# pecos/tps

Measured on AMD Instinct MI355X. Metric: DG RHS evals/sec (MDOF/s) for 3D p=3 reacting cyl at 1/2/4/8 MI355X, higher is better.
Workload: dtype f64

## Files before the change

### include/tpsrhs.h

```cpp
#ifndef TPSRHS_H_
#define TPSRHS_H_

#include <stdint.h>

#ifdef __cplusplus
extern "C" {
#endif

#define TPSRHS_MAXDIM 3
#define TPSRHS_MAXSPECIES 8
#define TPSRHS_MAXEQUATIONS (TPSRHS_MAXDIM + 2 + TPSRHS_MAXSPECIES)
#define TPSRHS_MAXREACTIONS 34
#define TPSRHS_MAXCHEMPARAMS 3
#define TPSRHS_MAXTABLE 1000
#define TPSRHS_MAXORDER 5

enum tpsrhs_status {
  TPSRHS_OK = 0,
  TPSRHS_ERR_INVALID_ARGUMENT = 1,
  TPSRHS_ERR_UNSUPPORTED = 2,
  TPSRHS_ERR_MESH = 3,
  TPSRHS_ERR_DEVICE = 4,
  TPSRHS_ERR_NO_DEVICE = 5,
  TPSRHS_ERR_HALO = 6
// ... 148 lines not shown
} tpsrhs_chemistry;

typedef struct tpsrhs_radiation {
  int model;
  tpsrhs_table nec_table;
} tpsrhs_radiation;

enum tpsrhs_sgs_model { TPSRHS_SGS_NONE = 0, TPSRHS_SGS_SMAGORINSKY = 1, TPSRHS_SGS_SIGMA = 2 };
typedef struct tpsrhs_sgs {
  int model_type;
  double model_const;
  double model_floor;
} tpsrhs_sgs;
typedef struct tpsrhs_visc_sponge {
  int enabled;
  double normal[3], point[3];
  double width, ratio;
} tpsrhs_visc_sponge;

typedef struct tpsrhs_lte {
  tpsrhs_table energy_table;
  tpsrhs_table gas_constant_table;
  tpsrhs_table sound_speed_table;
  tpsrhs_table viscosity_table;
  tpsrhs_table conductivity_table;
  tpsrhs_table electric_conductivity_table;
} tpsrhs_lte;

typedef struct tpsrhs_physics {
  int eq_system;
  int working_fluid;
  tpsrhs_dry_air dry_air;
  tpsrhs_perfect_mixture mixture;
  int transport_model;
  tpsrhs_constant_transport constant_transport;
  tpsrhs_gas_transport gas_transport;
  tpsrhs_chemistry chemistry;
  tpsrhs_radiation radiation;
  tpsrhs_sgs sgs;
  tpsrhs_visc_sponge visc_sponge;
  tpsrhs_lte lte;
} tpsrhs_physics;

typedef struct tpsrhs_bc {
  int attribute;
  int category;
  int type;
  double data[4 + TPSRHS_MAXSPECIES];
} tpsrhs_bc;

typedef int (*tpsrhs_halo_fn)(void *ctx, int phase, const double *send, double *recv,
                              int num_neighbors, const int *neighbor_ranks,
                              const int64_t *send_offsets, const int64_t *recv_offsets, void *stream);

enum tpsrhs_reduce_op { TPSRHS_REDUCE_SUM = 0, TPSRHS_REDUCE_MIN = 1 };
typedef int (*tpsrhs_reduce_fn)(void *ctx, double *values, int count, int op, void *stream);

typedef struct tpsrhs_runtime {
  int device;
  void *stream;
  tpsrhs_halo_fn halo;
  void *halo_ctx;
  tpsrhs_reduce_fn reduce;
  void *reduce_ctx;
} tpsrhs_runtime;

typedef struct tpsrhs_operator *tpsrhs_handle;

int tpsrhs_create(const tpsrhs_mesh *mesh, const tpsrhs_disc *disc, const tpsrhs_physics *physics,
                  int num_bcs, const tpsrhs_bc *bcs, const tpsrhs_runtime *runtime,
                  tpsrhs_handle *out);

int tpsrhs_destroy(tpsrhs_handle h);

int tpsrhs_mult(tpsrhs_handle h, const double *x, double *y, double time, double *max_char_speed);

int tpsrhs_mult_host(tpsrhs_handle h, const double *x, double *y, double time,
                     double *max_char_speed);

int tpsrhs_update_gradients(tpsrhs_handle h, const double *x);

int tpsrhs_get_primitives(tpsrhs_handle h, double *up_out);
int tpsrhs_get_gradients(tpsrhs_handle h, double *gradup_out);
int tpsrhs_get_plasma_conductivity(tpsrhs_handle h, const double *x, double *sigma_out);

enum tpsrhs_point_quantity {
  TPSRHS_POINT_PRIMITIVES = 0,
  TPSRHS_POINT_PRESSURE = 1,
  TPSRHS_POINT_SOUND_SPEED = 2,
  TPSRHS_POINT_MAX_CHAR_SPEED = 3
};
int tpsrhs_eval_pointwise(tpsrhs_handle h, int quantity, int64_t n, const double *U, double *out);

int tpsrhs_table_eval(const tpsrhs_table *table, int64_t n, const double *x, double *f);

int tpsrhs_math_eval(int function, int64_t n, const double *x, double *y);

int64_t tpsrhs_height(tpsrhs_handle h);
int64_t tpsrhs_num_dofs(tpsrhs_handle h);
int tpsrhs_num_equation(tpsrhs_handle h);

int tpsrhs_enable_kernel_timing(tpsrhs_handle h, int enable);
int tpsrhs_kernel_times(tpsrhs_handle h, int capacity, const char **names, double *milliseconds);
int tpsrhs_mult_times(tpsrhs_handle h, int capacity, double *milliseconds);

int tpsrhs_kernel_bytes(tpsrhs_handle h, int capacity, const char **names, double *bytes);

int tpsrhs_rk4_step(tpsrhs_handle h, double *x, double *time, double dt, double *max_char_speed, int64_t *nan_count);

int tpsrhs_advance(tpsrhs_handle h, double *x, double *time, double *dt, int num_steps, int constant_dt, double cfl,
                   double hmin, int64_t *nan_count);

int tpsrhs_set_dt(tpsrhs_handle h, double dt);

#define TPSRHS_MAXHEATSOURCES 4
#define TPSRHS_MAXSPONGEZONES 2
#define TPSRHS_MAXPASSIVESCALARS 4

typedef struct tpsrhs_heat_source {
  double value;
  double radius, point1[3], point2[3];
} tpsrhs_heat_source;

enum tpsrhs_sponge_type { TPSRHS_SPONGE_PLANAR = 0, TPSRHS_SPONGE_ANNULUS = 1 };
enum tpsrhs_sponge_solution { TPSRHS_SPONGE_USERDEF = 0, TPSRHS_SPONGE_MIXEDOUT = 1 };

typedef struct tpsrhs_sponge_zone {
  int type;
  int solution_type;
  double tol;
  double normal[3], point0[3], point_init[3];
  double r1, r2;
  double mult_factor;
  double target_U[TPSRHS_MAXEQUATIONS];
} tpsrhs_sponge_zone;

typedef struct tpsrhs_passive_scalar {
  double coords[3];
  double radius;
  double value;
} tpsrhs_passive_scalar;

typedef struct tpsrhs_forcing {
  int has_pressure_gradient;
  double pressure_gradient[3];
  int num_heat_sources;
  tpsrhs_heat_source heat_sources[TPSRHS_MAXHEATSOURCES];
  int num_sponge_zones;
  tpsrhs_sponge_zone sponge_zones[TPSRHS_MAXSPONGEZONES];
  int num_passive_scalars;
  tpsrhs_passive_scalar passive_scalars[TPSRHS_MAXPASSIVESCALARS];
} tpsrhs_forcing;

int tpsrhs_set_forcing(tpsrhs_handle h, const tpsrhs_forcing *forcing);

typedef struct tpsrhs_mixing_length {
  double max_mixing_length;
  double pr_ratio;
  double lewis;
  double bulk_multiplier;
} tpsrhs_mixing_length;
int tpsrhs_set_mixing_length(tpsrhs_handle h, const double *distance, const tpsrhs_mixing_length *params);

int tpsrhs_set_joule_heating(tpsrhs_handle h, const double *joule_heating);

int tpsrhs_face_tables(const tpsrhs_mesh *mesh, int num_bcs, const tpsrhs_bc *bcs, int32_t *face_nbr,
// ... 11 lines not shown
```

### tps_amd/capi.py

```python
from __future__ import annotations

import ctypes as C
import os

import numpy as np

MAXDIM = 3
MAXSPECIES = 8
MAXEQUATIONS = MAXDIM + 2 + MAXSPECIES
MAXREACTIONS = 34
MAXCHEMPARAMS = 3
NUM_GASPARAMS = 4

EULER, NS, NS_PASSIVE = 0, 1, 2
DRY_AIR, USER_DEFINED, LTE_FLUID = 0, 1, 2
ARGON_MINIMAL, ARGON_MIXTURE, CONSTANT = 0, 1, 2
ARRHENIUS, HOFFERTLIEN, TABULATED_RXN = 0, 1, 2
NONE_RAD, NET_EMISSION = 0, 1
SPECIES_MW, SPECIES_CHARGES, FORMATION_ENERGY, SPECIES_DEGENERACY = 0, 1, 2, 3
CLMB_ATT, CLMB_REP, AR_AR1P, AR_E, AR_AR, NONE_ARGCOLL = 0, 1, 2, 3, 4, 5
INLET, OUTLET, WALL = 0, 1, 2
SUB_DENS_VEL, SUB_DENS_VEL_NR, SUB_VEL_CONST_ENT = 2, 6, 7
SUB_DENS_VEL_FACE_X, SUB_DENS_VEL_FACE_Y, SUB_DENS_VEL_FACE_Z = 3, 4, 5
SUB_P, SUB_P_NR, SUB_MF_NR, SUB_MF_NR_PW = 0, 2, 3, 4
# ... 452 lines not shown
    for sp in range(nsp):
        mx.gas_params[sp + SPECIES_MW * nsp] = mw[sp]
        mx.gas_params[sp + SPECIES_CHARGES * nsp] = -1.0 if sp == 3 else 0.0
        mx.gas_params[sp + FORMATION_ENERGY * nsp] = 0.0
        mx.gas_params[sp + SPECIES_DEGENERACY * nsp] = 1.0
        mx.molar_cv[sp] = cv[sp]
    ph.transport_model = CONSTANT
    ph.constant_transport.electron_index = 3
    ph.chemistry.electron_index = 3
    ph.chemistry.num_reactions = 0
    ph._keep = []
    return ph


def make_bc(attribute, category, bc_type, data=()) -> BC:
    bc = BC()
    bc.attribute, bc.category, bc.type = attribute, category, bc_type
    for i, v in enumerate(data):
        bc.data[i] = float(v)
    return bc


class MeshArgs:

    def __init__(self, hm):
        self.ev = np.ascontiguousarray(hm.elem_vertices, dtype=np.int32)
        self.ex = np.ascontiguousarray(hm.elem_coords, dtype=np.float64)
        self.bv = np.ascontiguousarray(hm.bdr_vertices, dtype=np.int32)
        self.ba = np.ascontiguousarray(hm.bdr_attributes, dtype=np.int32)
        m = Mesh()
        m.dim = hm.dim
        m.num_vertices = hm.num_vertices
        m.num_elements = hm.num_elements
        m.elem_vertices = self.ev.ctypes.data_as(_ip)
        m.elem_coords = self.ex.ctypes.data_as(_dp)
        m.num_bdr_faces = int(self.bv.shape[0])
        m.bdr_vertices = self.bv.ctypes.data_as(_ip)
        m.bdr_attributes = self.ba.ctypes.data_as(_ip)
        if hm.shared_vertices is not None and len(hm.shared_vertices):
            self.sv = np.ascontiguousarray(hm.shared_vertices, dtype=np.int32)
            self.sr = np.ascontiguousarray(hm.shared_neighbor_rank, dtype=np.int32)
            m.num_shared_faces = int(self.sv.shape[0])
            m.shared_vertices = self.sv.ctypes.data_as(_ip)
            m.shared_neighbor_rank = self.sr.ctypes.data_as(_ip)
        else:
            m.num_shared_faces = 0
        if getattr(hm, "elem_size", None) is not None:
            self.es = np.ascontiguousarray(hm.elem_size, dtype=np.float64)
            m.elem_size = self.es.ctypes.data_as(_dp)
        self.c = m


_LIB = None
LIB_PATH = os.environ.get("TPSRHS_LIB") or os.path.join(os.path.dirname(os.path.abspath(__file__)), "csrc", "libtpsrhs.so")


class LibraryMissing(RuntimeError):
    pass


def load():
    global _LIB
    if _LIB is not None:
        return _LIB
    if not os.path.exists(LIB_PATH):
        raise LibraryMissing(
            f"{LIB_PATH} not found: build it with `python -c 'import __graft_entry__ as g; g.build()'`. "
            "tps_amd has no CPU fallback.")
    import torch

    lib = C.CDLL(LIB_PATH)
    vp = C.c_void_p
    lib.tpsrhs_create.restype = C.c_int
    lib.tpsrhs_create.argtypes = [C.POINTER(Mesh), C.POINTER(Disc), C.POINTER(Physics), C.c_int, C.POINTER(BC),
                                  C.POINTER(Runtime), C.POINTER(vp)]
    lib.tpsrhs_destroy.argtypes = [vp]
    lib.tpsrhs_mult.restype = C.c_int
    lib.tpsrhs_mult.argtypes = [vp, vp, vp, C.c_double, _dp]
    lib.tpsrhs_mult_host.restype = C.c_int
    lib.tpsrhs_mult_host.argtypes = [vp, vp, vp, C.c_double, _dp]
    lib.tpsrhs_update_gradients.argtypes = [vp, vp]
    lib.tpsrhs_get_primitives.argtypes = [vp, vp]
    lib.tpsrhs_get_gradients.argtypes = [vp, vp]
    lib.tpsrhs_get_plasma_conductivity.argtypes = [vp, vp, vp]
    lib.tpsrhs_height.restype = C.c_int64
    lib.tpsrhs_height.argtypes = [vp]
    lib.tpsrhs_num_dofs.restype = C.c_int64
    lib.tpsrhs_num_dofs.argtypes = [vp]
    lib.tpsrhs_num_equation.argtypes = [vp]
    lib.tpsrhs_enable_kernel_timing.argtypes = [vp, C.c_int]
    lib.tpsrhs_kernel_times.argtypes = [vp, C.c_int, C.POINTER(C.c_char_p), _dp]
    lib.tpsrhs_mult_times.argtypes = [vp, C.c_int, _dp]
    lib.tpsrhs_eval_pointwise.argtypes = [vp, C.c_int, C.c_int64, vp, vp]
    lib.tpsrhs_table_eval.argtypes = [C.POINTER(Table), C.c_int64, vp, vp]
    lib.tpsrhs_math_eval.argtypes = [C.c_int, C.c_int64, vp, vp]
    lib.tpsrhs_kernel_bytes.argtypes = [vp, C.c_int, C.POINTER(C.c_char_p), _dp]
    lib.tpsrhs_rk4_step.argtypes = [vp, C.c_void_p, _dp, C.c_double, _dp, C.POINTER(C.c_int64)]
    lib.tpsrhs_advance.argtypes = [vp, C.c_void_p, _dp, _dp, C.c_int, C.c_int, C.c_double, C.c_double,
                                   C.POINTER(C.c_int64)]
    lib.tpsrhs_set_dt.argtypes = [vp, C.c_double]
    lib.tpsrhs_set_forcing.argtypes = [vp, C.POINTER(Forcing)]
    lib.tpsrhs_set_joule_heating.argtypes = [vp, C.c_void_p]
    lib.tpsrhs_set_mixing_length.argtypes = [vp, C.c_void_p, C.POINTER(MixingLength)]
    lib.tpsrhs_face_tables.restype = C.c_int
    lib.tpsrhs_face_tables.argtypes = [C.POINTER(Mesh), C.c_int, C.POINTER(BC), vp, vp, vp, vp]
    lib.tpsrhs_status_string.restype = C.c_char_p
    lib.tpsrhs_status_string.argtypes = [C.c_int]
    lib.tpsrhs_last_error.restype = C.c_char_p
    lib.tpsrhs_version.restype = C.c_char_p
    _LIB = lib
    return lib


EXPORTED_SYMBOLS = [
    "tpsrhs_create", "tpsrhs_destroy", "tpsrhs_mult", "tpsrhs_mult_host", "tpsrhs_update_gradients",
    "tpsrhs_get_primitives", "tpsrhs_get_gradients", "tpsrhs_get_plasma_conductivity", "tpsrhs_height", "tpsrhs_num_dofs", "tpsrhs_num_equation",
    "tpsrhs_enable_kernel_timing", "tpsrhs_kernel_times", "tpsrhs_mult_times", "tpsrhs_kernel_bytes",
    "tpsrhs_eval_pointwise", "tpsrhs_table_eval", "tpsrhs_math_eval", "tpsrhs_face_tables",
    "tpsrhs_rk4_step", "tpsrhs_advance", "tpsrhs_set_dt", "tpsrhs_set_forcing", "tpsrhs_set_joule_heating", "tpsrhs_set_mixing_length", "tpsrhs_status_string",
    "tpsrhs_last_error", "tpsrhs_version",
]


def face_tables(host_mesh, bcs=()):
    lib = load()
    ma = MeshArgs(host_mesh)
    nlf = 2 * host_mesh.dim
    ne = host_mesh.num_elements
    ns = ma.c.num_shared_faces
    fn = np.zeros(ne * nlf, dtype=np.int32)
    fo = np.zeros(ne * nlf, dtype=np.uint8)
    ss = np.zeros(max(ns, 1), dtype=np.int32)
    so = np.zeros(max(ns, 1), dtype=np.uint8)
    arr = (BC * max(1, len(bcs)))(*bcs)
    st = lib.tpsrhs_face_tables(C.byref(ma.c), len(bcs), arr, fn.ctypes.data, fo.ctypes.data, ss.ctypes.data,
                                so.ctypes.data)
    if st != 0:
        raise RuntimeError(f"tpsrhs_face_tables: {lib.tpsrhs_status_string(st).decode()}: "
                           f"{lib.tpsrhs_last_error().decode()}")
    return fn.reshape(ne, nlf), fo.reshape(ne, nlf), ss[:ns], so[:ns]
```

### tps_amd/csrc/kernels.hpp

```cpp
#ifndef TPSRHS_KERNELS_HPP_
#define TPSRHS_KERNELS_HPP_

#include <hip/hip_runtime.h>

#include <type_traits>

#include "basis.hpp"
#include "physics_dryair.hpp"

namespace tpsrhs {

#ifndef TPSRHS_MINW_GRAD
#define TPSRHS_MINW_GRAD 1
#endif
#ifndef TPSRHS_MINW_FLUX
#define TPSRHS_MINW_FLUX 3
#endif
#ifndef TPSRHS_NT_STORES
#define TPSRHS_NT_STORES 0
#endif
#ifndef TPSRHS_NO_MFMA
#define TPSRHS_NO_MFMA 0
#endif
#ifndef TPSRHS_FLUX_LATE
#define TPSRHS_FLUX_LATE 0
#endif
#ifndef TPSRHS_ABLATE
#define TPSRHS_ABLATE 0
#endif
#ifndef TPSRHS_LEAN_GENERAL
#define TPSRHS_LEAN_GENERAL 0
#endif
constexpr int cmax(int a, int b) { return a > b ? a : b; }

#ifndef TPSRHS_STAMP
#define TPSRHS_STAMP 0
#endif
#if TPSRHS_STAMP
constexpr int NSTAMP = 16, STAMP_BLOCKS = 1 << 16;
static __device__ unsigned int g_stamp[STAMP_BLOCKS][NSTAMP];
struct Stamper {
  unsigned long long t0;
  unsigned int acc[NSTAMP];
  __device__ inline unsigned long long now() {
    unsigned long long t;
    __builtin_amdgcn_sched_barrier(0);
    asm volatile("s_memtime %0\n\ts_waitcnt lgkmcnt(0)" : "=s"(t)::"memory");
    __builtin_amdgcn_sched_barrier(0);
    return t;
  }
  __device__ inline void start() {
    for (int i = 0; i < NSTAMP; i++) acc[i] = 0;
    t0 = now();
  }
  __device__ inline void mark(int phase) {
    const unsigned long long t = now();
    acc[phase] += static_cast<unsigned int>(t - t0);
    t0 = t;
  }
  __device__ inline void flush() {
    if (threadIdx.x == 0 && blockIdx.x < STAMP_BLOCKS)
      for (int i = 0; i < NSTAMP; i++) g_stamp[blockIdx.x][i] = acc[i];
  }
};
#endif
#ifndef TPSRHS_DUMPF
#define TPSRHS_DUMPF 0
#endif
#if TPSRHS_DUMPF
constexpr int DUMPF_MAX = 1 << 22;
static __device__ double g_dumpf[DUMPF_MAX];
#endif
#if TPSRHS_STAMP == 1
#define STAMP_DECL Stamper stamper
#define STAMP_ARG , stamper
#define STAMP_PARAM , Stamper &stamper
#define STAMP_START() stamper.start()
#define STAMP(phase) stamper.mark(phase)
#define STAMP_FLUSH() stamper.flush()
#else
#define STAMP_DECL
#define STAMP_ARG
#define STAMP_PARAM
#define STAMP_START()
#define STAMP(phase)
#define STAMP_FLUSH()
#endif
#if TPSRHS_STAMP == 2
#define FSTAMP_DECL \
  Stamper stamper;  \
  stamper.start()
#define FSTAMP(phase) stamper.mark(phase)
#define FSTAMP_FLUSH() stamper.flush()
#else
#define FSTAMP_DECL
#define FSTAMP(phase)
#define FSTAMP_FLUSH()
#endif

static __constant__ Tables1D c_tab[2][2][TPSRHS_MAXORDER + 1];

__device__ inline const Tables1D &fresh_table(const Tables1D &ct) {
  typedef const Tables1D __attribute__((address_space(4))) *CP;
  const unsigned long long a = reinterpret_cast<unsigned long long>(&ct);
  unsigned lo = __builtin_amdgcn_readfirstlane(static_cast<unsigned>(a));
  unsigned hi = __builtin_amdgcn_readfirstlane(static_cast<unsigned>(a >> 32));
  asm volatile("" : "+s"(lo), "+s"(hi));
  return *(const Tables1D *)reinterpret_cast<CP>((static_cast<unsigned long long>(hi) << 32) | lo);
}

__device__ inline double ldsr(const double *p) { return *p; }

__device__ inline const double *field_ptr(const double *base, int k, int64_t stride) { return base + k * stride; }
__device__ inline double *field_ptr(double *base, int k, int64_t stride) { return base + k * stride; }
// ... 6 lines not shown
    __builtin_amdgcn_fence(__ATOMIC_ACQUIRE, "wavefront");
  } else {
    __syncthreads();
  }
}

template <int DIM_, int P_, int NC_ = 0>
struct Cfg {
  static constexpr int DIM = DIM_, P = P_, N1 = P_ + 1, NC = NC_;
  static constexpr int NPE = (DIM_ == 3) ? N1 * N1 * N1 : N1 * N1;
  static constexpr int NF = (DIM_ == 3) ? N1 * N1 : N1;
  static constexpr int Q1 = ((DIM_ - 1) + 2 * P_) / 2 + 1 + NC_;
  static constexpr int QV = P_ + 1 + NC_;
  static constexpr int NQV = (DIM_ == 3) ? QV * QV * QV : QV * QV;
  static constexpr int NQ = (DIM_ == 3) ? Q1 * Q1 : Q1;
  static constexpr int NW = (DIM_ == 3) ? Q1 * N1 : 1;
  static constexpr int NFACES = 2 * DIM_;
  static constexpr int NV = 1 << DIM_;
  static constexpr int BLOCK = (NC_ && DIM_ == 3 && P_ >= 2) ? 128 : ((NPE <= 64) ? 64 : ((NPE <= 128) ? 128 : 256));
  static constexpr int EPB = (DIM_ == 3 && NC_) ? (P_ == 3 ? 1 : 2)
                             : (DIM_ == 3 && P_ == 1) ? 3
                             : (DIM_ == 2 && NC_ && P_ == 1) ? 10
                                                             : BLOCK / NPE;
  static constexpr int NODES = EPB * NPE;
  static constexpr int PF = 2 * EPB;
  static constexpr int TN = PF * NF;
  static constexpr int TW = PF * NW;
  static constexpr int TQ = PF * NQ;
  static constexpr int LN = EPB * NF;
  static constexpr int Q_ROUNDS = (TQ + BLOCK - 1) / BLOCK;
  static_assert(DIM_ == 2 || Q_ROUNDS == 1, "3-D: one round of face quadrature points per direction pair");
  static_assert(!(DIM_ == 2 && NC_) || Q_ROUNDS == 1, "2-D Gauss-Lobatto pair: one round per direction pair");
  static constexpr int TQ2 = 2 * TQ;
  static constexpr int Q2_ROUNDS = (TQ2 + BLOCK - 1) / BLOCK;
};

template <class C>
struct Tab {
  double x[C::N1], w[C::N1], iw[C::N1], D[C::N1 * C::N1], b0[C::N1], b1[C::N1];
  double xq[C::Q1], wq[C::Q1], B[C::Q1 * C::N1];
  double xv[C::QV], wv[C::QV];
};

struct ForcingDev {
  int has_pg, nheat, nsponge, pad;
  double pg[3];
  struct Heat {
    double value, radius, len;
    double p1[3], axis[3];
  } heat[TPSRHS_MAXHEATSOURCES];
  struct Sponge {
    int type, pad;
    double normal[3], p0[3], pinit[3];
    double r1, r2, mult;
    double target[TPSRHS_MAXEQUATIONS];
    int mixed_out, n_plane;
    const int *plane_nodes;
    double *msum;
  } sponge[TPSRHS_MAXSPONGEZONES];
  const double *joule;
  int nps, pad2;
  struct Scalar {
    double x0[3], radius, value;
  } ps[TPSRHS_MAXPASSIVESCALARS];
};

struct RkDev {
  int mode, sp_first, sp_last, pad;
  double dt_host;
  const double *dt_dev;
  const double *x0, *y2, *y3, *y4;
  double *out;
  unsigned long long *nan_count;
  double *ta_out;
};

struct MeshDev {
  const int *blocks;
  int ne;
  int reverse;
  int64_t ndofs;
  const double *verts;
  const int2 *face_info;
  const double *minv;
  MixLenDev ml;
  VsDev vs;
};
__device__ inline EddyCtx closure_ctx(const MeshDev &m, bool dist_on, double dist, const double *X, double *park) {
  EddyCtx ec = dist_on ? eddy_at(m.ml, dist) : eddy_off();
  if (m.vs.enabled) {
    park[threadIdx.x] = visc_sponge_weight_2d(m.vs, X);
    ec.vsw = park;
  }
  return ec;
}

#ifndef TPSRHS_GRAD_LATE
#define TPSRHS_GRAD_LATE 1
#endif
#ifndef TPSRHS_GRAD_LATE_NC
#define TPSRHS_GRAD_LATE_NC 0
#endif
#ifndef TPSRHS_FLUX_PARK_GRAD
#define TPSRHS_FLUX_PARK_GRAD 0
#endif
#ifndef TPSRHS_GRAD_LATE_ALL
#define TPSRHS_GRAD_LATE_ALL 0
#endif
#ifndef TPSRHS_XCD_ORDER
#define TPSRHS_XCD_ORDER 1
#endif
__device__ inline int xcd_block(int b, int n, int reverse = 0) {
#if TPSRHS_XCD_ORDER
  constexpr int X = 8;
  const int q = n / X, r = n - q * X;
  const int x = b % X, k = b / X;
  const int kk = reverse ? (q + (x < r ? 1 : 0)) - 1 - k : k;
  return x * q + (x < r ? x : r) + kk;
#else
  return reverse ? n - 1 - b : b;
#endif
}

template <class C>
__device__ inline void load_face_info(int2 *sFI, const MeshDev &m, int e0) {
  for (int i = threadIdx.x; i < C::EPB * C::NFACES; i += C::BLOCK) {
    const int e = e0 + i / C::NFACES;
    sFI[i] = (e < m.ne) ? m.face_info[static_cast<int64_t>(e0) * C::NFACES + i] : make_int2(INT32_MIN, 0);
  }
}

template <class C>
__device__ constexpr int stride_of(int d) {
  return d == 0 ? 1 : (d == 1 ? C::N1 : C::N1 * C::N1);
}
template <class C>
__device__ constexpr int tan_a(int d) {
  return (C::DIM == 2) ? 1 - d : ((d == 0) ? 1 : 0);
}
template <class C>
__device__ constexpr int tan_b(int d) {
  return (d == 2) ? 1 : 2;
}
template <int DIM>
__device__ inline int permute(int o, int n, int ia, int ib) {
  const int fa = (o >> 1) & 1, fb = (o >> 2) & 1;
  if (DIM == 2) return fa ? n - 1 - ia : ia;
  int ja, jb;
  if (!(o & 1)) {
    ja = fa ? n - 1 - ia : ia;
    jb = fb ? n - 1 - ib : ib;
  } else {
    ja = fa ? n - 1 - ib : ib;
    jb = fb ? n - 1 - ia : ia;
  }
  return ja + n * jb;
}

template <int DIM>
__device__ inline void jacobian(const double *V, const double *xi, double *J) {
  if (DIM == 2) {
    const double x = xi[0], y = xi[1];
#pragma unroll
    for (int i = 0; i < 2; i++) {
      const double v00 = V[0 * 2 + i], v10 = V[1 * 2 + i], v01 = V[2 * 2 + i], v11 = V[3 * 2 + i];
      J[i + 0 * 2] = (v10 - v00) * (1.0 - y) + (v11 - v01) * y;
      J[i + 1 * 2] = (v01 - v00) * (1.0 - x) + (v11 - v10) * x;
    }
  } else {
    const double x = xi[0], y = xi[1], z = xi[2];
// ... 712 lines not shown
    const int item = tid + rd * C::BLOCK;
#pragma unroll
    for (int eq = 0; eq < NEQ; eq++) jump[rd][eq] = 0.0;
#pragma unroll
    for (int d = 0; d < DIM; d++) nw[rd][d] = 0.0;
    if (item < C::TQ) {
      const int pf = item / C::NQ, q = item - pf * C::NQ;
      const int le = pf >> 1, s = pf & 1;
      const int nb = sFI[le * C::NFACES + 2 * D + s].x;
      if (nb != INT32_MIN) {
        double bq[C::N1];
        const int qrow = (DIM == 2) ? q : q / C::Q1;
#pragma unroll
        for (int a = 0; a < C::N1; a++) bq[a] = tab.B[qrow * C::N1 + a];
        double u1[NEQ], u2[NEQ];
#pragma unroll
        for (int eq = 0; eq < NEQ; eq++) {
          u1[eq] = interp2_point<C>(sT + eq * C::TN, Wb + eq * C::TW, bq, pf, q);
          u2[eq] = interp2_point<C>(sT + (NEQ + eq) * C::TN, Wb + (NEQ + eq) * C::TW, bq, pf, q);
        }
        if (nb < 0) {
#pragma unroll
          for (int eq = 0; eq < NEQ; eq++) u2[eq] = u1[eq];
          if (prm.use_bc_in_grad) PH::bc_grad_prim(prm, prm.bc[-nb - 1], u1, u2);
        }
        double n[DIM], wq, Xq[DIM];
        face_geometry<C, D>(&sV[le * C::NV * DIM], tab, s, q, n, wq, Xq);
#pragma unroll
        for (int eq = 0; eq < NEQ; eq++) jump[rd][eq] = 0.5 * (u2[eq] - u1[eq]);
#pragma unroll
        for (int d = 0; d < DIM; d++) nw[rd][d] = wq * n[d];
      }
    }
  }
  block_sync<C::BLOCK>();
#pragma unroll
  for (int d = 0; d < DIM; d++) {
#pragma unroll
    for (int rd = 0; rd < C::Q_ROUNDS; rd++) {
      const int item = tid + rd * C::BLOCK;
      if (item < C::TQ) {
#pragma unroll
        for (int eq = 0; eq < NEQ; eq++) R[eq * C::TQ + item] = nw[rd][d] * jump[rd][eq];
      }
    }
    block_sync<C::BLOCK>();
    double *W2 = (DIM == 3) ? Wb : R;
    project1_lines<C, NEQ>(R, Wb, ct, tid);
    if (DIM == 3) block_sync<C::BLOCK>();
    project2_lines<C, NEQ>(W2, sT, ct, tid);
    block_sync<C::BLOCK>();
    if (node_on) {
#pragma unroll
      for (int eq = 0; eq < NEQ; eq++) g[eq + d * NEQ] += lift_pair<C, D>(sT + eq * C::TN, tab, le_n, idx);
    }
    block_sync<C::BLOCK>();
  }
}

template <class C, class PH>
struct GradLds {
  static constexpr int NEQ = PH::NEQ, DIM = C::DIM;
  static constexpr int NVF = NEQ * (1 + DIM);
  static constexpr int CH = NEQ;
  static constexpr int SUP = cmax(NEQ * C::NODES, (DIM == 2 ? 2 : 1) * CH * C::TN);
  static constexpr bool LEAN3D = PH::LEAN_TRACE && DIM == 3 && !C::NC && C::BLOCK == 64 && C::Q_ROUNDS == 1;
  static constexpr bool G_IN_LDS = PH::HEAVY && !LEAN3D;
  static constexpr int J = cmax(2 * NEQ * C::TN, (G_IN_LDS ? DIM : 1) * NEQ * C::NODES);
  static constexpr int W = CH * C::TW;
  static constexpr int V = C::NC ? cmax(cmax(NcScratch<C>::TOTAL, 2 * NEQ * C::TW + NEQ * C::TQ), NEQ * DIM * C::NODES) : 0;
  static constexpr int O_U = 0, O_UP = NEQ * C::NODES, O_J = O_UP + SUP, O_W = O_J + J, O_V = O_W + W;
  static constexpr int TOTAL = O_V + V;
};

template <class C>
__device__ inline void face_normal_rt(int d, const double *V, int s, double ta, double tb, double *n) {
  if (d == 0)
    face_normal_at<C, 0>(V, s, ta, tb, n);
  else if (d == 1 || C::DIM == 2)
    face_normal_at<C, 1>(V, s, ta, tb, n);
  else
    face_normal_at<C, (C::DIM == 3 ? 2 : 0)>(V, s, ta, tb, n);
}
template <class C, class PH>
__device__ inline void grad_jump_nodal(int D, const int2 *sFI, typename PH::PRef prm, const double *Town,
                                       const double *Tnb, const double *sV, const Tab<C> &tab, int le_n, const int *idx,
                                       double inv_mass, double *g) {
  constexpr int NEQ = PH::NEQ, DIM = C::DIM;
  const int da = (DIM == 2) ? 1 - D : (D == 0 ? 1 : 0), db = (D == 2) ? 1 : 2;
  const int ia = idx[da], ib = (DIM == 3) ? idx[db] : 0;
  const int fn = (DIM == 2) ? ia : ia + C::N1 * ib;
  const double wf = (DIM == 2) ? tab.w[ia] : tab.w[ia] * tab.w[ib];
#pragma clang loop unroll(disable)
  for (int s = 0; s < 2; s++) {
    const int pf = 2 * le_n + s;
    const int nb = sFI[le_n * C::NFACES + 2 * D + s].x;
    double u1[NEQ], u2[NEQ];
#pragma unroll
    for (int eq = 0; eq < NEQ; eq++) {
      u1[eq] = ldsr(&Town[eq * C::TN + pf * C::NF + fn]);
      u2[eq] = ldsr(&Tnb[eq * C::TN + pf * C::NF + fn]);
    }
    if (nb < 0 && prm.use_bc_in_grad) PH::bc_grad_prim(prm, prm.bc[-nb - 1], u1, u2);
    double n[DIM];
    face_normal_rt<C>(D, &sV[le_n * C::NV * DIM], s, tab.x[ia], (DIM == 3) ? tab.x[ib] : 0.0, n);
    const double c = 0.5 * wf * inv_mass * (s ? tab.b1[idx[D]] : tab.b0[idx[D]]);
#pragma unroll
    for (int dd = 0; dd < DIM; dd++) {
      const double cn = c * n[dd];
#pragma unroll
      for (int eq = 0; eq < NEQ; eq++) g[eq + dd * NEQ] += cn * (u2[eq] - u1[eq]);
    }
  }
}

template <class C, class PH, int D>
__device__ inline void visc_interp_dir(const double *sU, const double *g, bool node_on, double *sJ, double *Tb, double *Wb,
                                       const Tab<C> &tab, const Tables1D &ct,
                                       double (&v)[C::Q_ROUNDS][GradLds<C, PH>::NVF], int tid) {
  constexpr int NEQ = PH::NEQ, DIM = C::DIM;
  constexpr int G0 = PH::VISC_USES_GRAD_RHO ? 0 : 1, NG = NEQ - G0;
  auto point_stage = [&](auto nfld_tag, int v0, const double *T, const double *W) {
    constexpr int NF_ = decltype(nfld_tag)::value;
#pragma unroll
    for (int rd = 0; rd < C::Q_ROUNDS; rd++) {
      const int item = tid + rd * C::BLOCK;
      if (item < C::TQ) {
        const int pf = item / C::NQ, q = item - pf * C::NQ;
        double bq[C::N1];
        const int qrow = (DIM == 2) ? q : q / C::Q1;
#pragma unroll
        for (int a = 0; a < C::N1; a++) bq[a] = tab.B[qrow * C::N1 + a];
#pragma unroll
        for (int k = 0; k < NF_; k++) v[rd][v0 + k] = interp2_point<C>(T + k * C::TN, W + k * C::TW, bq, pf, q);
      }
    }
  };
  trace_lines<C, D, NEQ>(sU, Tb, ct, tid);
  block_sync<C::BLOCK>();
  interp1_lines<C, NEQ>(Tb, Wb, ct, tid);
  if (DIM == 3) block_sync<C::BLOCK>();
  point_stage(std::integral_constant<int, NEQ>(), 0, Tb, Wb);
  block_sync<C::BLOCK>();
#pragma unroll
  for (int c = 1; c <= DIM; c++) {
    const double *src;
    if constexpr (GradLds<C, PH>::G_IN_LDS) {
      src = sJ + ((c - 1) * NEQ + G0) * C::NODES;
    } else {
      if (node_on) {
#pragma unroll
        for (int eq = G0; eq < NEQ; eq++) sJ[eq * C::NODES + tid] = g[eq + (c - 1) * NEQ];
      }
      block_sync<C::BLOCK>();
      src = sJ + G0 * C::NODES;
    }
    trace_lines<C, D, NG>(src, Tb, ct, tid);
    block_sync<C::BLOCK>();
    interp1_lines<C, NG>(Tb, Wb, ct, tid);
    if (DIM == 3) block_sync<C::BLOCK>();
    if (G0) {
#pragma unroll
      for (int rd = 0; rd < C::Q_ROUNDS; rd++) v[rd][c * NEQ] = 0.0;
    }
    point_stage(std::integral_constant<int, NG>(), c * NEQ + G0, Tb, Wb);
    block_sync<C::BLOCK>();
  }
}
template <class C>
__device__ inline void face_geometry_rt(int d, const double *verts, const Tab<C> &tab, int s, int q, double *n, double &wq,
                                        double *Xq) {
  if (d == 0)
    face_geometry<C, 0>(verts, tab, s, q, n, wq, Xq);
  else if (d == 1 || C::DIM == 2)
    face_geometry<C, 1>(verts, tab, s, q, n, wq, Xq);
  else
    face_geometry<C, (C::DIM == 3 ? 2 : 0)>(verts, tab, s, q, n, wq, Xq);
}
template <int ROUNDS>
struct FaceDist {
  bool on = false;
  double d[ROUNDS] = {};
};
template <class C, class PH, bool BOTH = false>
__device__ inline void visc_points(const MeshDev &m, const int2 *sFI, typename PH::PRef prm0, int e0, int d,
                                   double (&v)[BOTH ? C::Q2_ROUNDS : C::Q_ROUNDS][GradLds<C, PH>::NVF], const double *sV,
                                   const Tab<C> &tab, double *__restrict__ TB, int tid,
                                   const FaceDist<BOTH ? C::Q2_ROUNDS : C::Q_ROUNDS> &dq = FaceDist<BOTH ? C::Q2_ROUNDS : C::Q_ROUNDS>()) {
// ... 163 lines not shown
          for (int eq = 1; eq < NEQ; eq++) fn[eq] -= 0.5 * f[eq];
        }
      }
    }
    if (on) {
      const int slot = (e0 + le) * C::NFACES + 2 * d + s;
      double *out = TB + static_cast<int64_t>(slot) * ((NEQ - 1) * C::NQ) + q;
#pragma unroll
      for (int eq = 1; eq < NEQ; eq++) out[(eq - 1) * C::NQ] = fn[eq];
    }
    STAMP(8);
  }
}
template <class C, class PH, int D, int CD>
__device__ inline void lean_grad_chunk(const double *sJ, double *Tb, double *Wb, const Tab<C> &tab, const Tables1D &ct0,
                                       const double *n, double *gv, double *gn, int tid) {
  constexpr int NEQ = PH::NEQ, DIM = C::DIM, NVEL = PH::NVEL;
  const Tables1D &ct = fresh_table(ct0);
  trace_lines<C, D, NEQ>(sJ, Tb, ct, tid);
  block_sync<C::BLOCK>();
  interp1_lines<C, NEQ>(Tb, Wb, ct, tid);
  block_sync<C::BLOCK>();
  if (tid < C::TQ) {
    const int pf = tid / C::NQ, q = tid - pf * C::NQ;
    double bq[C::N1];
#pragma unroll
    for (int a = 0; a < C::N1; a++) bq[a] = tab.B[(q / C::Q1) * C::N1 + a];
#pragma unroll
    for (int k = 0; k < NEQ; k++) {
      const double val = interp2_point<C>(Tb + k * C::TN, Wb + k * C::TW, bq, pf, q);
      if (k >= 1 && k <= NVEL)
        gv[(k - 1) + CD * DIM] = val;
      else
        gn[k] += n[CD] * val;
    }
  }
  block_sync<C::BLOCK>();
}
template <class C, class PH, int D>
__device__ inline void lean_grad_dir(const MeshDev &m, const double *gradUp_q, bool node_on, unsigned node, double *gnext, double *sJ,
                                     double *Tb, double *Wb, const Tab<C> &tab, const Tables1D &ct, const double *n, double *gv,
                                     double *gn, int tid) {
  constexpr int NEQ = PH::NEQ;
  auto stage = [&](auto ctag) {
    constexpr int CD = decltype(ctag)::value;
    if (node_on) {
#pragma unroll
      for (int eq = 0; eq < NEQ; eq++) sJ[eq * C::NODES + tid] = gnext[eq];
      if (CD + 1 < C::DIM) {
        unsigned nq = node;
        int64_t stride = m.ndofs;
        asm volatile("" : "+v"(nq), "+s"(stride));
#pragma unroll
        for (int eq = 0; eq < NEQ; eq++) gnext[eq] = field_ptr(gradUp_q, (CD + 1) * NEQ + eq, stride)[nq];
      }
    }
    block_sync<C::BLOCK>();
    lean_grad_chunk<C, PH, D, CD>(sJ, Tb, Wb, tab, ct, n, gv, gn, tid);
  };
  stage(std::integral_constant<int, 0>());
  stage(std::integral_constant<int, 1>());
  stage(std::integral_constant<int, 2>());
}
template <class C, class PH>
__device__ inline void visc_phase_lean3d(const MeshDev &m, const int2 *sFI, typename PH::PRef prm0, int e0, const double *sU,
                                         const double *gradUp_q, bool node_on, unsigned node, double *sJ, double *Tb, double *Wb,
                                         const double *sV, const Tab<C> &tab, const Tables1D &ct, double *__restrict__ TB,
                                         int tid0 STAMP_PARAM) {
  constexpr int NEQ = PH::NEQ, DIM = C::DIM;
  static_assert(DIM == 3 && C::Q_ROUNDS == 1 && PH::NVEL == 3 && C::BLOCK == 64, "3-D, one wave, one round of face points per pair");
#pragma clang loop unroll(disable)
  for (int d = 0; d < DIM; d++) {
    typename PH::PRef prm = PH::relaunder(prm0);
    int tid = tid0;
    asm volatile("" : "+v"(tid));
    const int pf = tid / C::NQ, q = tid - pf * C::NQ;
    const int le = pf >> 1, s = pf & 1;
    const bool on = tid < C::TQ && (e0 + le) < m.ne;
    int nb = 0;
    double n[DIM] = {1.0, 0.0, 0.0};
    if (on) {
      double wq, Xq[DIM];
      nb = sFI[le * C::NFACES + 2 * d + s].x;
      face_geometry_rt<C>(d, &sV[le * C::NV * DIM], tab, s, q, n, wq, Xq);
    }
    const int np_lane = on ? PH::visc_passes(prm, nb) : 0;
    const int npass = (__ballot(np_lane == 2) != 0) ? 2 : ((__ballot(np_lane >= 1) != 0) ? 1 : 0);
    double *out = TB + static_cast<int64_t>((e0 + le) * C::NFACES + 2 * d + s) * ((NEQ - 1) * C::NQ) + q;
    if (on && np_lane == 0) {
#pragma unroll
      for (int eq = 1; eq < NEQ; eq++) out[(eq - 1) * C::NQ] = 0.0;
    }
#pragma clang loop unroll(disable)
    for (int pass = 0; pass < npass; pass++) {
      double u[NEQ];
#pragma unroll
      for (int k = 0; k < NEQ; k++) u[k] = 1.0;
      if (d == 0)
        visc_state_dir<C, PH, 0>(sU, Tb, Wb, tab, ct, u, tid);
      else if (d == 1)
        visc_state_dir<C, PH, 1>(sU, Tb, Wb, tab, ct, u, tid);
      else
        visc_state_dir<C, PH, 2>(sU, Tb, Wb, tab, ct, u, tid);
      STAMP(5);
      PH::clamp_species(u);
      double gnext[NEQ];
#pragma unroll
      for (int eq = 0; eq < NEQ; eq++) gnext[eq] = 0.0;
      if (node_on) {
        unsigned nq = node;
        int64_t stride = m.ndofs;
        asm volatile("" : "+v"(nq), "+s"(stride));
#pragma unroll
        for (int eq = 0; eq < NEQ; eq++) gnext[eq] = field_ptr(gradUp_q, eq, stride)[nq];
      }
      typename PH::ViscLean cf;
      if (pass < np_lane) {
        typename PH::PRef pq = PH::relaunder(prm);
        double Us[NEQ];
        typename PH::WallFlux w;
        PH::visc_pass_state(pq, nb, pass, u, n, Us, w);
        PH::visc_point_lean(pq, Us, w, cf);
      }
      STAMP(6);
      double gv[DIM * DIM], gn[NEQ];
#pragma unroll
      for (int k = 0; k < DIM * DIM; k++) gv[k] = 0.0;
#pragma unroll
      for (int eq = 0; eq < NEQ; eq++) gn[eq] = 0.0;
      if (d == 0)
        lean_grad_dir<C, PH, 0>(m, gradUp_q, node_on, node, gnext, sJ, Tb, Wb, tab, ct, n, gv, gn, tid);
      else if (d == 1)
        lean_grad_dir<C, PH, 1>(m, gradUp_q, node_on, node, gnext, sJ, Tb, Wb, tab, ct, n, gv, gn, tid);
      else
        lean_grad_dir<C, PH, 2>(m, gradUp_q, node_on, node, gnext, sJ, Tb, Wb, tab, ct, n, gv, gn, tid);
      STAMP(7);
      if (pass < np_lane) {
        double f[NEQ];
        PH::visc_normal_flux_lean(cf, gv, gn, n, f);
        if (nb >= 0) {
#pragma unroll
          for (int eq = 1; eq < NEQ; eq++) {
            if (TPSRHS_NT_STORES)
              __builtin_nontemporal_store(f[eq], &out[(eq - 1) * C::NQ]);
            else
              out[(eq - 1) * C::NQ] = f[eq];
          }
        } else if (pass == 0) {
#pragma unroll
          for (int eq = 1; eq < NEQ; eq++) out[(eq - 1) * C::NQ] = -0.5 * f[eq];
        } else {
#pragma unroll
          for (int eq = 1; eq < NEQ; eq++) out[(eq - 1) * C::NQ] -= 0.5 * f[eq];
        }
      }
      STAMP(8);
    }
    if (on && npass == 0) {
    }
  }
}
template <class C>
struct LeanLane {
  unsigned lane;
  unsigned tw;
  unsigned ir, iw;
  unsigned pw, pb;
// ... 71 lines not shown
  typedef const double __attribute__((address_space(1))) *GP;
#pragma unroll
  for (int eq = 0; eq < NEQ; eq++) {
    asm volatile("" : "+s"(a));
    gnext[eq] = reinterpret_cast<GP>(a)[lane];
    a += step;
  }
}
template <class C, class PH, int D>
__device__ inline void lean1_grad_dir(unsigned long long ga, unsigned long long gstep, bool node_on, double *gnext, double *sJ,
                                      double *Tb, double *Wb, const Tab<C> &tab, const Tables1D &ct0, const double *n, double *gv,
                                      double *gn, const LeanLane<C> &ll) {
  constexpr int NEQ = PH::NEQ, DIM = C::DIM, NVEL = PH::NVEL;
  const unsigned src = ll.template trace_src<D>();
  auto stage = [&](auto ctag) {
    constexpr int CD = decltype(ctag)::value;
    if (node_on) {
#pragma unroll
      for (int eq = 0; eq < NEQ; eq++) sJ[eq * C::NODES + ll.lane] = gnext[eq];
      if (CD + 1 < DIM) lean1_issue_grad<NEQ>(ga, gstep, ll.lane, gnext);
    }
    block_sync<C::BLOCK>();
    const Tables1D &ct = fresh_table(ct0);
    lean1_lines<C, D, NEQ>(sJ, Tb, Wb, ct, ll, src);
    double bq[C::N1];
#pragma unroll
    for (int a = 0; a < C::N1; a++) bq[a] = tab.B[ll.pb + a];
#pragma unroll
    for (int k = 0; k < NEQ; k++) {
      const double val = lean1_point<C>(Wb, k, bq, ll);
      if (k >= 1 && k <= NVEL)
        gv[(k - 1) + CD * DIM] = val;
      else if (CD == 0)
        gn[k] = 0.0 + n[CD] * val;
      else
        gn[k] += n[CD] * val;
    }
#pragma unroll
    for (int k = 0; k < NEQ; k++) {
      if (k >= 1 && k <= NVEL)
        asm volatile("" : "+v"(gv[(k - 1) + CD * DIM]));
      else
        asm volatile("" : "+v"(gn[k]));
    }
    block_sync<C::BLOCK>();
  };
  stage(std::integral_constant<int, 0>());
  stage(std::integral_constant<int, 1>());
  stage(std::integral_constant<int, 2>());
}
template <class C, class PH, int D>
__device__ inline void lean1_state_dir(const double *sU, double *Tb, double *Wb, const Tab<C> &tab, const Tables1D &ct0, double *u,
                                       const LeanLane<C> &ll) {
  const Tables1D &ct = fresh_table(ct0);
  lean1_lines<C, D, PH::NEQ>(sU, Tb, Wb, ct, ll, ll.template trace_src<D>());
  double bq[C::N1];
#pragma unroll
  for (int a = 0; a < C::N1; a++) bq[a] = tab.B[ll.pb + a];
#pragma unroll
  for (int k = 0; k < PH::NEQ; k++) u[k] = lean1_point<C>(Wb, k, bq, ll);
  block_sync<C::BLOCK>();
}
template <class C, class PH>
__device__ inline void visc_phase_lean1(const MeshDev &m, const int2 *sFI, typename PH::PRef prm0, int e0, const double *sU,
                                        const double *gradUp_q, bool node_on0, double *sJ, double *Tb, double *Wb,
                                        const double *sV, const Tab<C> &tab, const Tables1D &ct, double *__restrict__ TB,
                                        int tid0 STAMP_PARAM) {
  constexpr int NEQ = PH::NEQ, DIM = C::DIM;
  static_assert(DIM == 3 && C::Q_ROUNDS == 1 && PH::NVEL == 3 && C::BLOCK == 64 && C::EPB == 1, "3-D, one wave = one hex");
  const bool node_on = __builtin_amdgcn_readfirstlane(node_on0) != 0;
#pragma clang loop unroll(disable)
  for (int d = 0; d < DIM; d++) {
    typename PH::PRef prm = PH::relaunder(prm0);
    int tid = tid0;
    asm volatile("" : "+v"(tid));
    const int pf = tid / C::NQ, q = tid - pf * C::NQ;
    const int le = pf >> 1, s = pf & 1;
    const bool on = tid < C::TQ && (e0 + le) < m.ne;
    int nb = 0;
    double n[DIM] = {1.0, 0.0, 0.0};
    if (on) {
      double wq, Xq[DIM];
      nb = sFI[le * C::NFACES + 2 * d + s].x;
      face_geometry_rt<C>(d, &sV[le * C::NV * DIM], tab, s, q, n, wq, Xq);
    }
    const int np_lane = on ? PH::visc_passes(prm, nb) : 0;
    const int npass = (__ballot(np_lane == 2) != 0) ? 2 : ((__ballot(np_lane >= 1) != 0) ? 1 : 0);
    double *out = TB + static_cast<int64_t>((e0 + le) * C::NFACES + 2 * d + s) * ((NEQ - 1) * C::NQ) + q;
    if (on && np_lane == 0) {
#pragma unroll
      for (int eq = 1; eq < NEQ; eq++) out[(eq - 1) * C::NQ] = 0.0;
    }
#pragma clang loop unroll(disable)
    for (int pass = 0; pass < npass; pass++) {
      double u[NEQ];
      int tid1 = tid0;
      asm volatile("" : "+v"(tid1));
      const LeanLane<C> ll(static_cast<unsigned>(tid1) & (C::BLOCK - 1));
      if (d == 0)
        lean1_state_dir<C, PH, 0>(sU, Tb, Wb, tab, ct, u, ll);
      else if (d == 1)
        lean1_state_dir<C, PH, 1>(sU, Tb, Wb, tab, ct, u, ll);
      else
        lean1_state_dir<C, PH, 2>(sU, Tb, Wb, tab, ct, u, ll);
      STAMP(5);
      PH::clamp_species(u);
      double gnext[NEQ];
      unsigned long long ga = lean1_grad_base<C>(gradUp_q, e0);
      const unsigned long long gstep = static_cast<unsigned long long>(m.ndofs) * sizeof(double);
      if (node_on) {
        lean1_issue_grad<NEQ>(ga, gstep, ll.lane, gnext);
      } else {
#pragma unroll
        for (int eq = 0; eq < NEQ; eq++) gnext[eq] = 0.0;
      }
      typename PH::ViscLean cf;
      if (pass < np_lane) {
        typename PH::PRef pq = PH::relaunder(prm);
        double Us[NEQ];
        typename PH::WallFlux w;
        PH::visc_pass_state(pq, nb, pass, u, n, Us, w);
        PH::visc_point_lean(pq, Us, w, cf);
      }
      STAMP(6);
      double gv[DIM * DIM], gn[NEQ];
      if (d == 0)
        lean1_grad_dir<C, PH, 0>(ga, gstep, node_on, gnext, sJ, Tb, Wb, tab, ct, n, gv, gn, ll);
      else if (d == 1)
        lean1_grad_dir<C, PH, 1>(ga, gstep, node_on, gnext, sJ, Tb, Wb, tab, ct, n, gv, gn, ll);
      else
        lean1_grad_dir<C, PH, 2>(ga, gstep, node_on, gnext, sJ, Tb, Wb, tab, ct, n, gv, gn, ll);
      STAMP(7);
      if (pass < np_lane) {
        double f[NEQ];
        PH::visc_normal_flux_lean(cf, gv, gn, n, f);
        if (nb >= 0) {
#pragma unroll
          for (int eq = 1; eq < NEQ; eq++) {
            if (TPSRHS_NT_STORES)
              __builtin_nontemporal_store(f[eq], &out[(eq - 1) * C::NQ]);
            else
              out[(eq - 1) * C::NQ] = f[eq];
          }
        } else if (pass == 0) {
#pragma unroll
          for (int eq = 1; eq < NEQ; eq++) out[(eq - 1) * C::NQ] = -0.5 * f[eq];
        } else {
#pragma unroll
          for (int eq = 1; eq < NEQ; eq++) out[(eq - 1) * C::NQ] -= 0.5 * f[eq];
        }
      }
      STAMP(8);
    }
  }
}
template <class C, class PH>
__device__ inline void visc_phase_2d(const MeshDev &m, const int2 *sFI, typename PH::PRef prm, int e0,
                                     const double *sU, const double *g, bool node_on, double *sJ, double *Tb,
                                     const double *sV, const Tab<C> &tab, const Tables1D &ct, double *__restrict__ TB,
                                     int tid, const double *sDist = nullptr) {
  static_assert(C::DIM == 2, "2-D only");
  constexpr int NEQ = PH::NEQ;
  typedef GradLds<C, PH> L;
  constexpr int G0 = PH::VISC_USES_GRAD_RHO ? 0 : 1, NG = NEQ - G0;
  double v[C::Q2_ROUNDS][L::NVF];
  auto chunk = [&](auto nfld_tag, const double *src, int v0) {
    constexpr int NF_ = decltype(nfld_tag)::value;
    trace_lines<C, 0, NF_>(src, Tb, ct, tid);
    trace_lines<C, 1, NF_>(src, Tb + L::CH * C::TN, ct, tid);
    block_sync<C::BLOCK>();
#pragma unroll
    for (int rd = 0; rd < C::Q2_ROUNDS; rd++) {
      int item = tid + rd * C::BLOCK;
      if (item < C::TQ2) {
        const int d = item / C::TQ;
        item -= d * C::TQ;
        const int pf = item / C::NQ, q = item - pf * C::NQ;
        const double *T = Tb + d * (L::CH * C::TN);
        double bq[C::N1];
#pragma unroll
        for (int a = 0; a < C::N1; a++) bq[a] = tab.B[q * C::N1 + a];
#pragma unroll
        for (int k = 0; k < NF_; k++) v[rd][v0 + k] = interp2_point<C>(T + k * C::TN, nullptr, bq, pf, q);
      }
    }
    block_sync<C::BLOCK>();
  };
  chunk(std::integral_constant<int, NEQ>(), sU, 0);
  FaceDist<C::Q2_ROUNDS> dq;
  dq.on = sDist != nullptr;
  if (sDist) {
    trace_lines<C, 0, 1>(sDist, Tb, ct, tid);
    trace_lines<C, 1, 1>(sDist, Tb + L::CH * C::TN, ct, tid);
    block_sync<C::BLOCK>();
#pragma unroll
    for (int rd = 0; rd < C::Q2_ROUNDS; rd++) {
      int item = tid + rd * C::BLOCK;
      dq.d[rd] = 0.0;
      if (item < C::TQ2) {
        const int d = item / C::TQ;
        item -= d * C::TQ;
        const int pf = item / C::NQ, q = item - pf * C::NQ;
        double bq[C::N1];
#pragma unroll
        for (int a = 0; a < C::N1; a++) bq[a] = tab.B[q * C::N1 + a];
        dq.d[rd] = interp2_point<C>(Tb + d * (L::CH * C::TN), nullptr, bq, pf, q);
      }
    }
    block_sync<C::BLOCK>();
  }
#pragma unroll
  for (int c = 1; c <= 2; c++) {
    const double *src;
    if constexpr (L::G_IN_LDS) {
      src = sJ + ((c - 1) * NEQ + G0) * C::NODES;
    } else {
      if (node_on) {
#pragma unroll
        for (int eq = G0; eq < NEQ; eq++) sJ[eq * C::NODES + tid] = g[eq + (c - 1) * NEQ];
      }
      block_sync<C::BLOCK>();
      src = sJ + G0 * C::NODES;
    }
    if (G0) {
#pragma unroll
      for (int rd = 0; rd < C::Q2_ROUNDS; rd++) v[rd][c * NEQ] = 0.0;
    }
    chunk(std::integral_constant<int, NG>(), src, c * NEQ + G0);
  }
  visc_points<C, PH, true>(m, sFI, prm, e0, 0, v, sV, tab, TB, tid, dq);
}
template <class C, class PH, int D>
__device__ inline void visc_traces_dir(const MeshDev &m, const int2 *sFI, typename PH::PRef prm, int e0,
                                       const double *sU, const double *g, bool node_on, double *sJ, double *Tb, double *Wb,
                                       const double *sV, const Tab<C> &tab, const Tables1D &ct, double *__restrict__ TB,
                                       int tid) {
  double v[C::Q_ROUNDS][GradLds<C, PH>::NVF];
  visc_interp_dir<C, PH, D>(sU, g, node_on, sJ, Tb, Wb, tab, ct, v, tid);
  visc_points<C, PH>(m, sFI, prm, e0, D, v, sV, tab, TB, tid);
}

template <class C, class PH>
__global__ __launch_bounds__(C::BLOCK, (C::NC && PH::HEAVY) ? 1 : PH::minw_grad(C::DIM, C::P, C::NC)) void k_gradient(MeshDev m, typename PH::KArg prm_k,
                                                       const double *__restrict__ U, const double *__restrict__ TA,
                                                       double *__restrict__ Upout, double *__restrict__ gradUp,
                                                       double *__restrict__ TB) {
  typename PH::PRef prm = PH::pref(prm_k);
  constexpr int NEQ = PH::NEQ, DIM = C::DIM;
  typedef GradLds<C, PH> L;
  const Tables1D &ct = c_tab[C::NC][DIM - 2][C::P];
  __shared__ Tab<C> tab;
  __shared__ double sV[C::EPB * C::NV * DIM];
  __shared__ double pool[L::TOTAL];
  double *sU = pool + L::O_U;
  double *sUp = pool + L::O_UP;
  double *sJ = pool + L::O_J;
  double *sW = pool + L::O_W;

  const int tid = threadIdx.x;
  const int lin = xcd_block(static_cast<int>(blockIdx.x), static_cast<int>(gridDim.x), m.reverse);
  const int bid = m.blocks ? m.blocks[lin] : lin;
  const int e0 = (TPSRHS_ABLATE & 512) ? (bid % 8) * C::EPB : bid * C::EPB;
  __shared__ int2 sFI[C::EPB * C::NFACES];
  STAMP_DECL;
  STAMP_START();
  const bool node_on = tid < C::NODES && (e0 + tid / C::NPE) < m.ne;
  const int le_n = tid / C::NPE, nd = tid - le_n * C::NPE;
  int idx[3] = {nd % C::N1, (nd / C::N1) % C::N1, nd / (C::N1 * C::N1)};
  double u[NEQ];
  if (node_on) {
    const unsigned n = static_cast<unsigned>(e0 + le_n) * C::NPE + nd;
#pragma unroll
    for (int eq = 0; eq < NEQ; eq++) u[eq] = field_ptr(U, eq, m.ndofs)[n];
  }
  load_face_info<C>(sFI, m, e0);
  load_tables<C>(tab, ct);
  load_vertices<C>(sV, m, e0);
  block_sync<C::BLOCK>();
  STAMP(0);
  NbTraces<C, NEQ> ta0, ta1, ta2;
  constexpr bool LATE = TPSRHS_GRAD_LATE && ((DIM == 3 && (!C::NC || TPSRHS_GRAD_LATE_NC) && !PH::HEAVY) || TPSRHS_GRAD_LATE_ALL);
  issue_neighbour_traces<C, 0, NEQ>(sFI, TA, 2 * NEQ * C::NF, NEQ, ta0, tid);
  if (!LATE) {
    issue_neighbour_traces<C, 1, NEQ>(sFI, TA, 2 * NEQ * C::NF, NEQ, ta1, tid);
    if (DIM == 3) issue_neighbour_traces<C, (DIM == 3 ? 2 : 0), NEQ>(sFI, TA, 2 * NEQ * C::NF, NEQ, ta2, tid);
  }
  if (node_on) {
    const unsigned n = static_cast<unsigned>(e0 + le_n) * C::NPE + nd;
    double up[NEQ];
    PH::prim(prm, u, up);
#pragma unroll
    for (int eq = 0; eq < NEQ; eq++) {
      sU[eq * C::NODES + tid] = u[eq];
      sUp[eq * C::NODES + tid] = up[eq];
      if (TPSRHS_NT_STORES)
        __builtin_nontemporal_store(up[eq], &field_ptr(Upout, eq, m.ndofs)[n]);
      else
        field_ptr(Upout, eq, m.ndofs)[n] = up[eq];
    }
  }
  block_sync<C::BLOCK>();
  STAMP(1);

  double g[NEQ * DIM];
#pragma unroll
  for (int k = 0; k < NEQ * DIM; k++) g[k] = 0.0;
  double inv_mass = 0.0;
  if constexpr (C::NC) {
    nc_volume_gradient<C, NEQ>(sUp, pool + L::O_V, sV, tab, ct, node_on, le_n, nd, tid, g);
  } else if (node_on) {
    double xi[DIM], J[DIM * DIM], A[DIM * DIM];
    double iwn = 1.0;
#pragma unroll
    for (int d = 0; d < DIM; d++) {
      xi[d] = tab.x[idx[d]];
      iwn *= tab.iw[idx[d]];
    }
    jacobian<DIM>(&sV[le_n * C::NV * DIM], xi, J);
    const double det = adjugate<DIM>(J, A);
    const double idet = fast_rcp(det);
    inv_mass = iwn * idet;
    double Dr[DIM][C::N1];
#pragma unroll
    for (int mm = 0; mm < DIM; mm++)
#pragma unroll
      for (int a = 0; a < C::N1; a++) Dr[mm][a] = tab.D[idx[mm] * C::N1 + a];
#pragma unroll
    for (int eq = 0; eq < NEQ; eq++) {
      double dr[DIM];
#pragma unroll
      for (int mm = 0; mm < DIM; mm++) {
        const int m2 = ((TPSRHS_ABLATE & 128) && DIM == 3) ? 2 : mm;
        const int sd = stride_of<C>(m2);
        const double *F = &sUp[eq * C::NODES + le_n * C::NPE + nd - idx[m2] * sd];
        double acc = 0.0;
#pragma unroll
        for (int a = 0; a < C::N1; a++) acc += Dr[mm][a] * ldsr(&F[a * sd]);
        dr[mm] = acc;
      }
#pragma unroll
      for (int d = 0; d < DIM; d++) {
        double s = 0.0;
#pragma unroll
        for (int mm = 0; mm < DIM; mm++) s += A[mm + d * DIM] * dr[mm];
        g[eq + d * NEQ] = s * idet;
      }
    }
  }

  STAMP(2);
  if (!(TPSRHS_ABLATE & 8)) {
    auto jump = [&](auto dtag) {
      constexpr int D = decltype(dtag)::value;
      if constexpr (C::NC) {
        nc_grad_jump<C, PH, D>(sFI, prm, sJ, pool + L::O_V, sV, tab, ct, node_on, le_n, idx, tid, g);
      } else {
        if (node_on) grad_jump_nodal<C, PH>(D, sFI, prm, sJ, sJ + NEQ * C::TN, sV, tab, le_n, idx, inv_mass, g);
        block_sync<C::BLOCK>();
      }
    };
    if (LATE) issue_neighbour_traces<C, 1, NEQ>(sFI, TA, 2 * NEQ * C::NF, NEQ, ta1, tid);
    trace_lines<C, 0, NEQ>(sUp, sJ, ct, tid);
    block_sync<C::BLOCK>();
    store_neighbour_traces<C, NEQ>(ta0, sJ, sJ + NEQ * C::TN, tid);
    block_sync<C::BLOCK>();
    jump(std::integral_constant<int, 0>());
    if (LATE && DIM == 3) issue_neighbour_traces<C, (DIM == 3 ? 2 : 0), NEQ>(sFI, TA, 2 * NEQ * C::NF, NEQ, ta2, tid);
    trace_lines<C, 1, NEQ>(sUp, sJ, ct, tid);
    block_sync<C::BLOCK>();
    store_neighbour_traces<C, NEQ>(ta1, sJ, sJ + NEQ * C::TN, tid);
    block_sync<C::BLOCK>();
    jump(std::integral_constant<int, 1>());
    if (DIM == 3) {
      trace_lines<C, (DIM == 3 ? 2 : 0), NEQ>(sUp, sJ, ct, tid);
      block_sync<C::BLOCK>();
      store_neighbour_traces<C, NEQ>(ta2, sJ, sJ + NEQ * C::TN, tid);
      block_sync<C::BLOCK>();
      jump(std::integral_constant<int, (DIM == 3 ? 2 : 0)>());
    }
  }
  if constexpr (C::NC) {
    if constexpr (C::NPE == 64 && C::BLOCK == 128 && !TPSRHS_NO_MFMA) {
      static_assert(L::V >= 64 * 17, "LDS buffer of the MFMA inverse mass");
      nc_apply_minv_mfma<C, NEQ * DIM>(m.minv, pool + L::O_V, node_on, e0, nd, tid, g);
    }
    else
      nc_apply_minv<C, NEQ * DIM>(m.minv, pool + L::O_V, node_on, e0 + le_n, le_n, nd, tid, g);
  }

  STAMP(3);
  if (node_on) {
    const unsigned n = static_cast<unsigned>(e0 + le_n) * C::NPE + nd;
#pragma unroll
    for (int k = 0; k < NEQ * DIM; k++) field_ptr(gradUp, k, m.ndofs)[n] = g[k];
    if constexpr (L::G_IN_LDS) {
#pragma unroll
      for (int k = 0; k < NEQ * DIM; k++) sJ[k * C::NODES + tid] = g[k];
    }
  }
  if (L::G_IN_LDS) block_sync<C::BLOCK>();
  STAMP(4);
  if constexpr (L::LEAN3D) {
    if (!(TPSRHS_ABLATE & 16)) {
      asm volatile("s_waitcnt vmcnt(0)" ::: "memory");
      const double *gq = gradUp;
      const unsigned node = static_cast<unsigned>(e0 + le_n) * C::NPE + nd;
      if constexpr (PH::LEAN_ONE_HEX && C::EPB == 1 && C::BLOCK % C::LN == 0 && !TPSRHS_ABLATE && !TPSRHS_LEAN_GENERAL)
        visc_phase_lean1<C, PH>(m, sFI, prm, e0, sU, gq, node_on, sJ, sUp, sW, sV, tab, ct, TB, tid STAMP_ARG);
      else
        visc_phase_lean3d<C, PH>(m, sFI, prm, e0, sU, gq, node_on, node, sJ, sUp, sW, sV, tab, ct, TB, tid STAMP_ARG);
    }
    STAMP_FLUSH();
    return;
  }

  if (!(TPSRHS_ABLATE & 16)) {
    if constexpr (DIM == 2) {
      if constexpr (PH::HEAVY) {
        __shared__ double sDist[C::NODES];
        const bool ml_on = m.ml.distance != nullptr;
        if (ml_on) {
          if (tid < C::NODES)
            sDist[tid] = node_on ? m.ml.distance[static_cast<int64_t>(e0 + le_n) * C::NPE + nd] : 0.0;
          block_sync<C::BLOCK>();
        }
        visc_phase_2d<C, PH>(m, sFI, prm, e0, sU, g, node_on, sJ, sUp, sV, tab, ct, TB, tid, ml_on ? sDist : nullptr);
      } else {
        visc_phase_2d<C, PH>(m, sFI, prm, e0, sU, g, node_on, sJ, sUp, sV, tab, ct, TB, tid);
      }
    } else if constexpr (PH::TWO_STEP && C::Q_ROUNDS == 1 && !(TPSRHS_ABLATE & 256)) {
      visc_phase_heavy3d<C, PH>(m, sFI, prm, e0, sU, sJ, sUp, sW, sV, tab, ct, TB, tid STAMP_ARG);
    } else if constexpr (PH::HEAVY) {
#pragma clang loop unroll(disable)
      for (int d = 0; d < DIM; d++) {
        double v[C::Q_ROUNDS][L::NVF];
        if (d == 0)
          visc_interp_dir<C, PH, 0>(sU, g, node_on, sJ, sUp, sW, tab, ct, v, tid);
        else if (d == 1)
          visc_interp_dir<C, PH, 1>(sU, g, node_on, sJ, sUp, sW, tab, ct, v, tid);
        else
          visc_interp_dir<C, PH, (DIM == 3 ? 2 : 0)>(sU, g, node_on, sJ, sUp, sW, tab, ct, v, tid);
        visc_points<C, PH>(m, sFI, prm, e0, d, v, sV, tab, TB, tid);
      }
    } else {
      visc_traces_dir<C, PH, 0>(m, sFI, prm, e0, sU, g, node_on, sJ, sUp, sW, sV, tab, ct, TB, tid);
      visc_traces_dir<C, PH, 1>(m, sFI, prm, e0, sU, g, node_on, sJ, sUp, sW, sV, tab, ct, TB, tid);
      if (DIM == 3)
        visc_traces_dir<C, PH, (DIM == 3 ? 2 : 0)>(m, sFI, prm, e0, sU, g, node_on, sJ, sUp, sW, sV, tab, ct, TB, tid);
    }
  }
  STAMP_FLUSH();
}

template <class C, class PH>
// ... 256 lines not shown
      __syncthreads();
    }
    if (tid == 0) sz.msum[eq] = red[0];
    __syncthreads();
  }
  if (tid == 0) sz.msum[NEQ] = static_cast<double>(sz.n_plane);
}
template <class C, class PH>
__global__ void k_mixed_out_finish(typename PH::KArg prm_k, ForcingDev *fd, int z) {
  typename PH::PRef prm = PH::pref(prm_k);
  constexpr int NEQ = PH::NEQ;
  ForcingDev::Sponge &sz = fd->sponge[z];
  double mean[NEQ], tgt[NEQ];
#pragma unroll
  for (int eq = 0; eq < NEQ; eq++) mean[eq] = sz.msum[eq] / sz.msum[NEQ];
  PH::state_from_mean_flux(prm, mean, sz.normal, tgt);
#pragma unroll
  for (int eq = 0; eq < NEQ; eq++) sz.target[eq] = tgt[eq];
}

template <class C, class PH>
__global__ __launch_bounds__(256) void k_forcing(MeshDev m, typename PH::KArg prm_k, const ForcingDev *__restrict__ fd,
                                                 const double *__restrict__ U, const double *__restrict__ gradUp,
                                                 double *__restrict__ Y) {
  typename PH::PRef prm = PH::pref(prm_k);
  constexpr int NEQ = PH::NEQ, DIM = C::DIM;
  const Tables1D &ct = c_tab[C::NC][DIM - 2][C::P];
  const int64_t n = static_cast<int64_t>(blockIdx.x) * 256 + threadIdx.x;
  if (n >= m.ndofs) return;
  const int e = static_cast<int>(n / C::NPE), nd = static_cast<int>(n - static_cast<int64_t>(e) * C::NPE);
  const int idx[3] = {nd % C::N1, (nd / C::N1) % C::N1, nd / (C::N1 * C::N1)};
  double xi[DIM], X[DIM];
#pragma unroll
  for (int d = 0; d < DIM; d++) xi[d] = ct.x[idx[d]];
  position<DIM>(m.verts + static_cast<int64_t>(e) * C::NV * DIM, xi, X);
  double u[NEQ], gr[NEQ * DIM], src[NEQ];
#pragma unroll
  for (int eq = 0; eq < NEQ; eq++) {
    u[eq] = field_ptr(U, eq, m.ndofs)[n];
    src[eq] = 0.0;
  }
  if (fd->has_pg) {
#pragma unroll
    for (int d = 0; d < DIM; d++) gr[(1 + d) + d * NEQ] = field_ptr(gradUp, (1 + d) + d * NEQ, m.ndofs)[n];
  }
  const typename PH::State st = PH::make_state(prm, u);
  apply_forcing<C, PH>(*fd, prm, n, X, u, st, gr, src);
#pragma unroll
  for (int eq = 0; eq < NEQ; eq++)
    if (src[eq] != 0.0) field_ptr(Y, eq, m.ndofs)[n] += src[eq];
}

template <class C, class PH>
struct FluxLds {
  static constexpr int NEQ = PH::NEQ, DIM = C::DIM;
  static constexpr bool BOTH_2D = (DIM == 2) && (NEQ <= 8);
  static constexpr int X = BOTH_2D ? 4 * NEQ * C::TN : cmax(cmax(2 * NEQ * C::TN, NEQ * C::TQ), NEQ * C::TN);
  static constexpr int Y = BOTH_2D ? 2 * NEQ * C::TQ
                                   : cmax(cmax(2 * NEQ * C::TW, NEQ * C::TW), (DIM == 2) ? NEQ * C::TQ : 0);
  static constexpr int NCV = C::NC ? NcScratch<C>::TOTAL : 0;
  static constexpr int GF = cmax(NEQ * DIM * C::NODES + NCV, X + Y);
  static constexpr int TOTAL = NEQ * C::NODES + GF;
  static_assert(!C::NC || X >= NEQ * C::NODES, "staging of the inverse-mass vectors");
};

template <class C, class PH>
constexpr bool flux_fuses_traces() {
  return C::DIM == 3 && !C::NC && FluxLds<C, PH>::TOTAL >= 2 * PH::NEQ * C::NODES + 2 * PH::NEQ * C::TN;
}

template <class PH>
__device__ inline typename PH::PRef flux_params(typename PH::PRef p) {
  if constexpr (PH::LAUNDER_FLUX)
    return PH::relaunder(p);
  else
    return p;
}
template <class C, class PH, int D>
__device__ inline void face_flux_dir(const MeshDev &m, typename PH::PRef prm, int e0, const double *sU,
                                     double *X, double *Yb, const double *sV, const Tab<C> &tab, const Tables1D &ct,
                                     const NbTraces<C, PH::NEQ> &ta, const NbFlux<C, PH::NEQ> &tb, bool node_on,
                                     int le_n, const int *idx, double *z, int tid) {
  constexpr int NEQ = PH::NEQ, DIM = C::DIM;
  trace_lines<C, D, NEQ>(sU, X, ct, tid);
  block_sync<C::BLOCK>();
  store_neighbour_traces<C, NEQ>(ta, X, X + NEQ * C::TN, tid);
  block_sync<C::BLOCK>();
  interp1_lines<C, 2 * NEQ>(X, Yb, ct, tid);
  if (DIM == 3) block_sync<C::BLOCK>();
  double fh[C::Q_ROUNDS][NEQ];
#pragma unroll
  for (int rd = 0; rd < C::Q_ROUNDS; rd++) {
    const int item = tid + rd * C::BLOCK;
#pragma unroll
    for (int eq = 0; eq < NEQ; eq++) fh[rd][eq] = 0.0;
    const int nb = tb.nb[rd];
    if (nb == INT32_MIN) continue;
    const int pf = item / C::NQ, q = item - pf * C::NQ;
    const int le = pf >> 1, s = pf & 1;
    double bq[C::N1];
    const int qrow = (DIM == 2) ? q : q / C::Q1;
#pragma unroll
    for (int a = 0; a < C::N1; a++) bq[a] = tab.B[qrow * C::N1 + a];
    double u1[NEQ], u2[NEQ];
#pragma unroll
    for (int eq = 0; eq < NEQ; eq++) {
      u1[eq] = interp2_point<C>(X + eq * C::TN, Yb + eq * C::TW, bq, pf, q);
      u2[eq] = interp2_point<C>(X + (NEQ + eq) * C::TN, Yb + (NEQ + eq) * C::TW, bq, pf, q);
    }
    PH::clamp_species(u1);
    double n[DIM], wq, Xq[DIM];
    face_geometry<C, D>(&sV[le * C::NV * DIM], tab, s, q, n, wq, Xq);
    if (TPSRHS_ABLATE & 4) {
#pragma unroll
      for (int eq = 0; eq < NEQ; eq++) fh[rd][eq] = u1[eq] + u2[eq] * n[0];
    } else if (nb >= 0) {
      PH::clamp_species(u2);
      PH::riemann(prm, u1, u2, n, fh[rd]);
#pragma unroll
      for (int eq = 0; eq < NEQ; eq++) fh[rd][eq] -= 0.5 * (tb.own[rd][eq] - tb.nbv[rd][eq]);
    } else {
      double ug[NEQ];
      PH::bc_ghost(prm, prm.bc[-nb - 1], u1, n, ug, nr_state<C, PH>(prm, nb, (e0 + le) * C::NFACES + 2 * D + s, q));
      PH::riemann_bc(prm, prm.bc[-nb - 1], u1, ug, n, fh[rd]);
#pragma unroll
      for (int eq = 0; eq < NEQ; eq++) fh[rd][eq] += tb.own[rd][eq];
    }
    if (PH::AXISYM) wq *= Xq[0];
#pragma unroll
    for (int eq = 0; eq < NEQ; eq++) fh[rd][eq] *= wq;
  }
  block_sync<C::BLOCK>();
  double *R = (DIM == 2) ? Yb : X;
#pragma unroll
  for (int rd = 0; rd < C::Q_ROUNDS; rd++) {
    const int item = tid + rd * C::BLOCK;
    if (item < C::TQ) {
#pragma unroll
      for (int eq = 0; eq < NEQ; eq++) R[eq * C::TQ + item] = fh[rd][eq];
    }
  }
  block_sync<C::BLOCK>();
  project1_lines<C, NEQ>(X, Yb, ct, tid);
  if (DIM == 3) block_sync<C::BLOCK>();
  project2_lines<C, NEQ>(Yb, X, ct, tid);
  block_sync<C::BLOCK>();
  if (node_on) {
#pragma unroll
    for (int eq = 0; eq < NEQ; eq++) z[eq] -= lift_pair<C, D>(X + eq * C::TN, tab, le_n, idx);
  }
  block_sync<C::BLOCK>();
}

template <class C, int NEQ>
struct NbFlux2 {
  double own[C::Q2_ROUNDS][NEQ], nbv[C::Q2_ROUNDS][NEQ];
  int nb[C::Q2_ROUNDS];
};
template <class C, int NEQ>
__device__ inline void issue_visc_traces_2d(const int2 *sFI, int e0, const double *__restrict__ TB, NbFlux2<C, NEQ> &t,
                                            int tid) {
#pragma unroll
  for (int r = 0; r < C::Q2_ROUNDS; r++) {
    int item = tid + r * C::BLOCK;
    t.nb[r] = INT32_MIN;
#pragma unroll
    for (int k = 0; k < NEQ; k++) t.own[r][k] = t.nbv[r][k] = 0.0;
    if (item < C::TQ2) {
      const int d = item / C::TQ;
      item -= d * C::TQ;
      const int pf = item / C::NQ, q = item - pf * C::NQ;
      const int lslot = (pf >> 1) * C::NFACES + 2 * d + (pf & 1);
      const int2 fi = sFI[lslot];
      t.nb[r] = fi.x;
      if (fi.x != INT32_MIN && !(TPSRHS_ABLATE & 1)) {
        const double *o = TB + (static_cast<int64_t>(e0) * C::NFACES + lslot) * ((NEQ - 1) * C::NQ) + q;
#pragma unroll
        for (int k = 1; k < NEQ; k++) t.own[r][k] = o[(k - 1) * C::NQ];
        if (fi.x >= 0) {
          const int pq = permute<2>(fi.y, C::Q1, q, 0);
          const double *b2 = TB + static_cast<int64_t>(fi.x) * ((NEQ - 1) * C::NQ) + pq;
#pragma unroll
          for (int k = 1; k < NEQ; k++) t.nbv[r][k] = b2[(k - 1) * C::NQ];
        }
      }
    }
  }
}
template <class C, class PH>
__device__ inline void face_flux_2d(const MeshDev &m, typename PH::PRef prm0, int e0, const double *sU, double *X,
                                    double *Yb, const double *sV, const Tab<C> &tab, const Tables1D &ct,
                                    const NbTraces<C, PH::NEQ> &ta0, const NbTraces<C, PH::NEQ> &ta1,
                                    const NbFlux2<C, PH::NEQ> &tb, bool node_on, int le_n, const int *idx, double *z,
                                    int tid) {
  static_assert(C::DIM == 2, "2-D only");
// ... 50 lines not shown
#pragma unroll
  for (int rd = 0; rd < C::Q2_ROUNDS; rd++) {
    int item = tid + rd * C::BLOCK;
    if (item < C::TQ2) {
      const int d = item / C::TQ;
      item -= d * C::TQ;
#pragma unroll
      for (int eq = 0; eq < NEQ; eq++) Yb[(d * NEQ + eq) * C::TQ + item] = fh[rd][eq];
    }
  }
  block_sync<C::BLOCK>();
  project2_lines<C, NEQ>(Yb, X, ct, tid);
  project2_lines<C, NEQ>(Yb + NEQ * C::TQ, X + XS, ct, tid);
  block_sync<C::BLOCK>();
  if (node_on) {
#pragma unroll
    for (int eq = 0; eq < NEQ; eq++)
      z[eq] -= lift_pair<C, 0>(X + eq * C::TN, tab, le_n, idx) + lift_pair<C, 1>(X + XS + eq * C::TN, tab, le_n, idx);
  }
  block_sync<C::BLOCK>();
}

template <class C, class PH>
__global__ __launch_bounds__(C::BLOCK, (C::NC && (PH::HEAVY || PH::MINW_FLUX > 2)) ? (PH::HEAVY ? 1 : 2) : PH::MINW_FLUX) void k_flux(MeshDev m, typename PH::KArg prm_k, const double *__restrict__ U,
                                                   const double *__restrict__ gradUp, const double *__restrict__ TA,
                                                   const double *__restrict__ TB, double *__restrict__ Y,
                                                   double *__restrict__ block_speed, RkDev rk) {
  typename PH::PRef prm = PH::pref(prm_k);
  constexpr int NEQ = PH::NEQ, DIM = C::DIM;
  typedef FluxLds<C, PH> L;
  const Tables1D &ct = c_tab[C::NC][DIM - 2][C::P];
  __shared__ Tab<C> tab;
  __shared__ double sV[C::EPB * C::NV * DIM];
  __shared__ double pool[L::TOTAL];
  double *sU = pool;
  double *sGf = pool + NEQ * C::NODES;
  double *sX = sGf, *sY = sGf + L::X;

  const int tid = threadIdx.x;
  const int lin = xcd_block(static_cast<int>(blockIdx.x), static_cast<int>(gridDim.x), m.reverse);
  const int bid = m.blocks ? m.blocks[lin] : lin;
  const int e0 = (TPSRHS_ABLATE & 512) ? (bid % 8) * C::EPB : bid * C::EPB;
  __shared__ int2 sFI[C::EPB * C::NFACES];
  FSTAMP_DECL;
  const bool node_on = tid < C::NODES && (e0 + tid / C::NPE) < m.ne;
  const int le_n = tid / C::NPE, nd = tid - le_n * C::NPE;
  int idx[3] = {nd % C::N1, (nd / C::N1) % C::N1, nd / (C::N1 * C::N1)};
  double u[NEQ], gr[NEQ * DIM];
  if (node_on) {
    const unsigned n = static_cast<unsigned>(e0 + le_n) * C::NPE + nd;
#pragma unroll
    for (int eq = 0; eq < NEQ; eq++) u[eq] = field_ptr(U, eq, m.ndofs)[n];
#pragma unroll
    for (int k = 0; k < NEQ * DIM; k++) gr[k] = field_ptr(gradUp, k, m.ndofs)[n];
  }
  load_face_info<C>(sFI, m, e0);
  load_tables<C>(tab, ct);
  load_vertices<C>(sV, m, e0);
  block_sync<C::BLOCK>();
  FSTAMP(0);
  NbTraces<C, NEQ> ta0;
  NbFlux<C, NEQ> tb0;
  constexpr bool EARLY = !(DIM == 2 && NEQ > 8) && !TPSRHS_FLUX_LATE;
  if (EARLY) {
    issue_neighbour_traces<C, 0, NEQ>(sFI, TA, 2 * NEQ * C::NF, 0, ta0, tid);
    if (!L::BOTH_2D) issue_visc_traces<C, 0, NEQ>(sFI, e0, TB, tb0, tid);
  }
  constexpr bool PARK = TPSRHS_FLUX_PARK_GRAD && PH::TWO_STEP && !C::NC && DIM == 3;
  if (node_on) {
#pragma unroll
    for (int eq = 0; eq < NEQ; eq++) sU[eq * C::NODES + tid] = u[eq];
    if constexpr (PARK) {
#pragma unroll
      for (int k = 0; k < NEQ * DIM; k++) sGf[k * C::NODES + tid] = gr[k];
    }
  }
  block_sync<C::BLOCK>();
  FSTAMP(1);

  double inv_mass = 0.0, speed = 0.0;
  double src[NEQ];
#pragma unroll
  for (int eq = 0; eq < NEQ; eq++) src[eq] = 0.0;
  if (node_on) {
    double F[NEQ * DIM];
    double radius = 1.0;
    double Xn[DIM] = {};
    if constexpr (PH::AXISYM || (PH::HEAVY && DIM == 2)) {
      if (PH::AXISYM || m.vs.enabled) {
        double xi[DIM];
#pragma unroll
        for (int d = 0; d < DIM; d++) xi[d] = tab.x[idx[d]];
        position<DIM>(&sV[le_n * C::NV * DIM], xi, Xn);
      }
      if (PH::AXISYM) radius = Xn[0];
    }
    {
      double uc[NEQ];
#pragma unroll
      for (int eq = 0; eq < NEQ; eq++) uc[eq] = u[eq];
      PH::clamp_species(uc);
      const typename PH::State st = PH::make_state(prm, uc);
      speed = PH::max_char_speed(prm, uc, st);
      typename PH::FluxCoef fc;
      if constexpr (PH::TWO_STEP) PH::flux_coeffs(prm, uc, st, fc);
      if constexpr (PARK) {
        const double *pg = sGf + tid;
        asm volatile("" : "+v"(pg) : : "memory");
#pragma unroll
        for (int k = 0; k < NEQ * DIM; k++) gr[k] = pg[k * C::NODES];
      }
      if (PH::HAS_SOURCE) {
        double up[NEQ];
        PH::prim(prm, u, up);
        PH::source(prm, u, up, gr, src);
        if constexpr (PH::AXISYM) PH::axisym_source(prm, u, up, gr, radius, src);
      }

      if (TPSRHS_ABLATE & 2) {
#pragma unroll
        for (int k = 0; k < NEQ * DIM; k++) F[k] = uc[k % NEQ] + gr[k];
      } else {
        if constexpr (PH::HEAVY && DIM == 2) {
          const bool ml_on = m.ml.distance != nullptr;
          __shared__ double sVsw[C::BLOCK];
          const EddyCtx ec = closure_ctx(m, true, ml_on ? m.ml.distance[static_cast<int64_t>(e0 + le_n) * C::NPE + nd] : 0.0, Xn, sVsw);
          if constexpr (PH::TWO_STEP)
            PH::total_flux(prm, uc, st, fc, gr, PH::AXISYM ? radius : -1.0, F, ec);
          else
            PH::total_flux(prm, uc, st, gr, radius, F, ec);
        } else if constexpr (PH::TWO_STEP)
          PH::total_flux(prm, uc, st, fc, gr, PH::AXISYM ? radius : -1.0, F);
        else if constexpr (PH::AXISYM)
          PH::total_flux(prm, uc, st, gr, radius, F);
        else if constexpr (PH::LES) {
          PointCtx pc;
          double xn[DIM];
#pragma unroll
          for (int d = 0; d < DIM; d++) xn[d] = tab.x[idx[d]];
          position<DIM>(&sV[le_n * C::NV * DIM], xn, pc.X);
          pc.delta = prm.elem_delta[e0 + le_n];
          PH::total_flux(prm, uc, st, gr, F, &pc);
        } else
          PH::total_flux(prm, uc, st, gr, F);
      }
    }
    __builtin_amdgcn_sched_barrier(0);
    double xi[DIM], J[DIM * DIM], A[DIM * DIM];
    double wn = 1.0, iwn = 1.0;
#pragma unroll
    for (int d = 0; d < DIM; d++) {
      xi[d] = tab.x[idx[d]];
      wn *= tab.w[idx[d]];
      iwn *= tab.iw[idx[d]];
    }
    jacobian<DIM>(&sV[le_n * C::NV * DIM], xi, J);
    const double det = adjugate<DIM>(J, A);
    inv_mass = iwn * fast_rcp(det);
    if (PH::AXISYM) {
      inv_mass *= fast_rcp(radius);
      wn *= radius;
    }
    __builtin_amdgcn_sched_barrier(0);
    if constexpr (C::NC) {
#pragma unroll
      for (int k = 0; k < NEQ * DIM; k++) sGf[k * C::NODES + tid] = F[k];
    } else {
#pragma unroll
      for (int eq = 0; eq < NEQ; eq++)
#pragma unroll
        for (int mm = 0; mm < DIM; mm++) {
          double s = 0.0;
#pragma unroll
          for (int d = 0; d < DIM; d++) s += A[mm + d * DIM] * F[eq + d * NEQ];
          sGf[(eq + mm * NEQ) * C::NODES + tid] = wn * s;
        }
    }
  }
  {
    double v = speed;
#pragma unroll
    for (int off = 32; off > 0; off >>= 1) v = fmax(v, __shfl_xor(v, off));
    if (C::BLOCK == 64) {
      if (tid == 0) block_speed[bid] = v;
    } else {
      __shared__ double swave[C::BLOCK / 64];
      if ((tid & 63) == 0) swave[tid >> 6] = v;
      block_sync<C::BLOCK>();
      if (tid == 0) {
        double b = swave[0];
#pragma unroll
        for (int w = 1; w < C::BLOCK / 64; w++) b = fmax(b, swave[w]);
        block_speed[bid] = b;
      }
    }
  }
  block_sync<C::BLOCK>();
  FSTAMP(2);
#if TPSRHS_DUMPF
  if (tid < C::NODES) {
    constexpr int ROWS = NEQ * DIM + NEQ;
    if ((static_cast<int64_t>(bid) + 1) * ROWS * C::NODES <= DUMPF_MAX) {
      double *out = g_dumpf + static_cast<int64_t>(bid) * ROWS * C::NODES + tid;
      for (int k = 0; k < NEQ * DIM; k++) out[k * C::NODES] = sGf[k * C::NODES + tid];
#pragma unroll
      for (int eq = 0; eq < NEQ; eq++) out[(NEQ * DIM + eq) * C::NODES] = src[eq];
    }
  }
#endif

  double z[NEQ];
#pragma unroll
  for (int eq = 0; eq < NEQ; eq++) z[eq] = 0.0;
  if constexpr (C::NC) {
    static_assert(!PH::AXISYM, "the non-collocated variant is planar / 3-D");
    nc_volume_divergence<C, NEQ>(sGf, sGf + NEQ * DIM * C::NODES, sV, tab, ct, node_on, le_n, nd, tid, z);
  } else if (node_on) {
    double Dc[DIM][C::N1];
#pragma unroll
    for (int mm = 0; mm < DIM; mm++)
#pragma unroll
      for (int a = 0; a < C::N1; a++) Dc[mm][a] = tab.D[a * C::N1 + idx[mm]];
#pragma unroll
    for (int eq = 0; eq < NEQ; eq++) {
      double acc = 0.0;
#pragma unroll
      for (int mm = 0; mm < DIM; mm++) {
        const int m2 = ((TPSRHS_ABLATE & 128) && DIM == 3) ? 2 : mm;
        const int sd = stride_of<C>(m2);
        const double *F = &sGf[(eq + mm * NEQ) * C::NODES + le_n * C::NPE + nd - idx[m2] * sd];
#pragma unroll
        for (int a = 0; a < C::N1; a++) acc += Dc[mm][a] * ldsr(&F[a * sd]);
      }
      z[eq] = acc;
    }
  }
  block_sync<C::BLOCK>();
  FSTAMP(3);

  if constexpr (L::BOTH_2D) {
// ... 230 lines not shown
```

### tps_amd/csrc/operator.hpp

```cpp
#ifndef TPSRHS_OPERATOR_HPP_
#define TPSRHS_OPERATOR_HPP_

#include <hip/hip_runtime.h>

#include <cstdio>
#include <cstdlib>
#include <cstring>
#include <memory>
#include <stdexcept>
#include <string>
#include <vector>

#include "../../include/tpsrhs.h"
#include "basis.hpp"
#include "kernels.hpp"
#include "topology.hpp"

using namespace tpsrhs;

namespace {

struct DeviceError : std::runtime_error {
  explicit DeviceError(const std::string &s) : std::runtime_error(s) {}
};
struct Unsupported : std::runtime_error {
  explicit Unsupported(const std::string &s) : std::runtime_error(s) {}
};

#define HIP_CHECK(expr)                                                                                   \
  do {                                                                                                    \
    hipError_t _e = (expr);                                                                               \
    if (_e != hipSuccess)                                                                                 \
      throw DeviceError(std::string(#expr) + ": " + hipGetErrorString(_e) + " (" __FILE__ ":" + std::to_string(__LINE__) + ")"); \
  } while (0)

inline bool poison_allocations() {
  const char *e = std::getenv("TPSRHS_POISON");
  return e && e[0] == '1';
}
template <class T>
T *dev_alloc(size_t n) {
  T *p = nullptr;
  const size_t bytes = std::max<size_t>(n, 1) * sizeof(T);
  HIP_CHECK(hipMalloc(reinterpret_cast<void **>(&p), bytes));
  if (poison_allocations()) {
    HIP_CHECK(hipMemset(p, 0xFF, bytes));
    HIP_CHECK(hipDeviceSynchronize());
  }
  return p;
}
template <class T>
T *dev_upload(const std::vector<T> &v) {
  T *p = dev_alloc<T>(v.size());
  if (!v.empty()) HIP_CHECK(hipMemcpy(p, v.data(), v.size() * sizeof(T), hipMemcpyHostToDevice));
  return p;
}

constexpr int NKERN = 3;
const char *kKernelNames[NKERN] = {"k_traces", "k_gradient", "k_flux"};

}

struct tpsrhs_operator {
  int dim = 0, order = 0, neq = 0, nvel = 0;
  int nc = 0;
  double *d_minv = nullptr;
  int ne = 0, nfaces = 0, nf = 0, nq = 0;
  int64_t ndofs = 0;
  int device = 0;
  hipStream_t stream = nullptr;
  Topology topo;
  tpsrhs_physics phys;
  alignas(16) unsigned char params[4096];
  void *d_chem = nullptr;
  void *d_params = nullptr;
  std::vector<void *> d_extra;
  std::vector<void *> d_mixed_out;
  double *d_verts = nullptr;
  int2 *d_face_info = nullptr;
  double *d_Up = nullptr, *d_gradUp = nullptr, *d_TA = nullptr, *d_TB = nullptr;
  double *d_speed = nullptr, *d_block_speed = nullptr;
  int flux_grid = 0;
  double *d_xh = nullptr, *d_yh = nullptr;
  double *d_rk = nullptr;
  unsigned long long *d_nan = nullptr;
  RkDev rk = {};
  MixLenDev mixlen = {nullptr, 0.0, 1.0, 0.0};
  ForcingDev forcing = {};
  ForcingDev *d_forcing = nullptr;
  bool forcing_active = false;
  bool has_nr = false;
  int n_nr_faces = 0;
  int2 *d_nr_faces = nullptr;
  int *d_nr_ordinal = nullptr;
  double *d_bstate[2] = {nullptr, nullptr};
  int bstate_cur = 0;
  bool bstate_init = false;
  double *d_bc_sums = nullptr;
  double nr_dt = 0.0;
  double *d_ctl = nullptr;
  const double *nr_dt_dev = nullptr;
  tpsrhs_reduce_fn reduce = nullptr;
  void *reduce_ctx = nullptr;
  hipGraphExec_t step_graph = nullptr;
  struct StepKey {
    const void *x = nullptr;
    int constant_dt = 0, bstate_cur = 0, epoch = 0;
    double coef = 0.0;
    bool operator==(const StepKey &o) const {
      return x == o.x && constant_dt == o.constant_dt && bstate_cur == o.bstate_cur && epoch == o.epoch && coef == o.coef;
    }
  } step_key;
  int config_epoch = 0;
  tpsrhs_halo_fn halo = nullptr;
  void *halo_ctx = nullptr;
  hipStream_t comm_stream = nullptr;
  hipEvent_t ev_halo[4] = {};
  int *d_blocks_halo = nullptr, *d_blocks_interior = nullptr;
  int n_blocks_halo = 0, n_blocks_interior = 0;
  int32_t *d_shared_slot = nullptr;
  uint8_t *d_shared_orient = nullptr;
  double *d_send = nullptr;
  std::vector<int64_t> send_off[2], recv_off[2];
  static constexpr int MAXSETS = 128;
  bool timing = false;
  hipEvent_t evs[MAXSETS][NKERN + 1] = {};
  int64_t sets_recorded = 0;
  hipEvent_t *ev = evs[0];

  void (*launch)(tpsrhs_operator *, const double *, double *, bool) = nullptr;
  void (*point_eval)(tpsrhs_operator *, int, int64_t, const double *, double *) = nullptr;
  bool fuse_traces = true;
  bool ta_valid = false;
  bool ta_chain = false;
  double *d_TA2 = nullptr, *d_ta_next = nullptr;
  bool sweep_alt = true;
  int sweep_parity = 0;
  VsDev vs2d = {};

  MeshDev mesh_dev() const {
    MeshDev m;
    m.blocks = nullptr;
    m.ne = ne;
    m.reverse = 0;
    m.ndofs = ndofs;
    m.verts = d_verts;
    m.face_info = d_face_info;
    m.minv = d_minv;
    m.ml = mixlen;
    m.vs = vs2d;
    return m;
  }
  ~tpsrhs_operator() {
    (void)hipSetDevice(device);
    for (void *p : {static_cast<void *>(d_verts), static_cast<void *>(d_face_info),
                    static_cast<void *>(d_Up), static_cast<void *>(d_gradUp),
                    static_cast<void *>(d_TA), static_cast<void *>(d_TB), static_cast<void *>(d_speed), static_cast<void *>(d_block_speed),
                    static_cast<void *>(d_xh), static_cast<void *>(d_yh), static_cast<void *>(d_shared_slot),
                    static_cast<void *>(d_shared_orient), static_cast<void *>(d_send)})
      if (p) (void)hipFree(p);
    if (d_chem) (void)hipFree(d_chem);
    if (d_params) (void)hipFree(d_params);
    if (d_minv) (void)hipFree(d_minv);
    if (d_TA2) (void)hipFree(d_TA2);
    if (d_rk) (void)hipFree(d_rk);
    if (d_nan) (void)hipFree(d_nan);
    if (d_forcing) (void)hipFree(d_forcing);
    if (step_graph) (void)hipGraphExecDestroy(step_graph);
    for (void *p : {static_cast<void *>(d_nr_faces), static_cast<void *>(d_nr_ordinal), static_cast<void *>(d_bstate[0]),
                    static_cast<void *>(d_bstate[1]), static_cast<void *>(d_bc_sums), static_cast<void *>(d_ctl)})
      if (p) (void)hipFree(p);
    if (d_blocks_halo) (void)hipFree(d_blocks_halo);
    if (d_blocks_interior) (void)hipFree(d_blocks_interior);
    for (auto &e : ev_halo)
      if (e) (void)hipEventDestroy(e);
    if (comm_stream) (void)hipStreamDestroy(comm_stream);
    for (void *p : d_extra) (void)hipFree(p);
    for (void *p : d_mixed_out) (void)hipFree(p);
    for (auto &set : evs)
      for (auto &e : set)
        if (e) (void)hipEventDestroy(e);
  }
};

namespace {

template <class PH>
typename PH::KArg kernel_params(tpsrhs_operator *op) {
  if constexpr (std::is_pointer<typename PH::KArg>::value) {
    if (!op->d_params) {
      op->d_params = dev_alloc<unsigned char>(sizeof(op->params));
      HIP_CHECK(hipMemcpy(op->d_params, op->params, sizeof(op->params), hipMemcpyHostToDevice));
    }
    return reinterpret_cast<typename PH::KArg>(op->d_params);
  } else {
    return *reinterpret_cast<const typename PH::Params *>(op->params);
  }
}

inline void exchange(tpsrhs_operator *op, int phase, double *T, int nfld, int per, hipStream_t stream) {
  const Topology &tp = op->topo;
  if (tp.num_shared == 0) return;
  const int n1 = (phase == 0) ? op->order + 1 : rule_points(op->nc, (op->dim - 1) + 2 * op->order);
  const int64_t total = static_cast<int64_t>(tp.num_shared) * nfld * per;
  const int grid = static_cast<int>(std::min<int64_t>((total + 255) / 256, 2048));
  if (op->dim == 3)
    hipLaunchKernelGGL(k_pack<3>, dim3(grid), dim3(256), 0, stream, tp.num_shared, nfld, n1, op->d_shared_slot,
                       op->d_shared_orient, T, op->d_send);
  else
    hipLaunchKernelGGL(k_pack<2>, dim3(grid), dim3(256), 0, stream, tp.num_shared, nfld, n1, op->d_shared_slot,
                       op->d_shared_orient, T, op->d_send);
  HIP_CHECK(hipGetLastError());
  double *recv = T + static_cast<int64_t>(op->ne) * op->nfaces * nfld * per;
  const int st = op->halo(op->halo_ctx, phase, op->d_send, recv, static_cast<int>(tp.nbr_ranks.size()),
                          tp.nbr_ranks.data(), op->send_off[phase].data(), op->recv_off[phase].data(), stream);
  if (st != 0) throw std::runtime_error("halo callback failed in phase " + std::to_string(phase));
}

template <int DIM, int P, class PH, int NC = 0>
void launch_all(tpsrhs_operator *op, const double *x, double *y, bool gradients_only) {
  typedef Cfg<DIM, P, NC> C;
  static_assert(sizeof(typename PH::Params) <= sizeof(op->params), "parameter block too large");
  const typename PH::Params &prm = *reinterpret_cast<const typename PH::Params *>(op->params);
  const int nblocks = (op->ne + C::EPB - 1) / C::EPB;
  hipStream_t s = op->stream;
  if constexpr (PH::HAS_NR_BC) {
    typename PH::Params &w = *reinterpret_cast<typename PH::Params *>(op->params);
    w.bstate = op->d_bstate[op->bstate_cur];
    w.nr_ordinal = op->d_nr_ordinal;
    w.nr_dt = op->nr_dt;
  }
  const typename PH::KArg prm_k = kernel_params<PH>(op);
  if (!op->d_block_speed && !gradients_only) {
    op->d_block_speed = dev_alloc<double>(nblocks);
    op->flux_grid = nblocks;
  }
  const int dir0 = op->sweep_alt ? op->sweep_parity : 0;
  double *ta = op->d_TA;
  bool have_traces = false;
  if constexpr (flux_fuses_traces<C, PH>()) {
    const int stage = op->rk.mode;
    if ((stage >= 2 || (stage == 1 && op->ta_chain)) && op->ta_valid) {
      ta = op->d_ta_next;
      have_traces = true;
    }
    op->ta_valid = false;
    if (op->fuse_traces && !gradients_only && op->topo.num_shared == 0 && stage >= 1 && (stage <= 3 || op->ta_chain)) {
      if (!op->d_TA2) op->d_TA2 = dev_alloc<double>(static_cast<int64_t>(op->ne) * op->nfaces * 2 * PH::NEQ * C::NF);
      op->rk.ta_out = (ta == op->d_TA) ? op->d_TA2 : op->d_TA;
      op->d_ta_next = op->rk.ta_out;
      op->ta_valid = true;
    }
  } else {
    op->ta_valid = false;
  }
  auto traces = [&](MeshDev m, int grid) {
    if (have_traces) return;
    m.reverse = dir0;
    hipLaunchKernelGGL((k_traces<C, PH>), dim3(grid), dim3(C::BLOCK), 0, s, m, prm_k, x, ta);
    HIP_CHECK(hipGetLastError());
  };
  auto gradient = [&](MeshDev m, int grid) {
    m.reverse = op->sweep_alt ? 1 - dir0 : 0;
    hipLaunchKernelGGL((k_gradient<C, PH>), dim3(grid), dim3(C::BLOCK), 0, s, m, prm_k, x, ta, op->d_Up, op->d_gradUp,
                       op->d_TB);
    HIP_CHECK(hipGetLastError());
  };
  auto flux = [&](MeshDev m, int grid) {
    m.reverse = dir0;
    hipLaunchKernelGGL((k_flux<C, PH>), dim3(grid), dim3(C::BLOCK), 0, s, m, prm_k, x, op->d_gradUp, ta, op->d_TB, y,
                       op->d_block_speed, op->rk);
    HIP_CHECK(hipGetLastError());
  };
  auto nr_update = [&](const MeshDev &m) {
    if constexpr (PH::HAS_NR_BC) {
      if (!op->has_nr) return;
      const int nbc = prm.num_bcs;
      hipLaunchKernelGGL((k_bc_mean<C, PH>), dim3(nbc), dim3(256), 0, s, op->n_nr_faces, op->d_nr_faces, ta,
                         op->d_bc_sums);
      HIP_CHECK(hipGetLastError());
      if (op->reduce && op->topo.num_shared > 0) {
        const int st = op->reduce(op->reduce_ctx, op->d_bc_sums, nbc * (TPSRHS_MAXEQUATIONS + 1), TPSRHS_REDUCE_SUM, s);
        if (st != 0) throw std::runtime_error("halo: reduce callback failed");
      }
      if (op->n_nr_faces > 0) {
        hipLaunchKernelGGL((k_bc_nr<C, PH>), dim3(op->n_nr_faces), dim3(C::BLOCK), 0, s, m, prm_k, op->d_nr_faces, op->d_bc_sums, x,
                           op->d_Up, op->d_gradUp, op->d_bstate[op->bstate_cur], op->d_bstate[1 - op->bstate_cur],
                           op->bstate_init ? 0 : 1, op->nr_dt_dev);
        HIP_CHECK(hipGetLastError());
      }
    }
  };
  auto forcing = [&](const MeshDev &m) {
    if (!op->forcing_active) return;
    if constexpr (PH::HAS_MIXED_OUT) {
      for (int z = 0; z < op->forcing.nsponge; z++) {
        if (!op->forcing.sponge[z].mixed_out) continue;
        hipLaunchKernelGGL((k_mixed_out_sum<C, PH>), dim3(1), dim3(256), 0, s, op->ndofs, prm_k, op->d_forcing, z, x);
        HIP_CHECK(hipGetLastError());
        if (op->reduce && op->topo.num_shared > 0) {
          const int st = op->reduce(op->reduce_ctx, op->forcing.sponge[z].msum, PH::NEQ + 1, TPSRHS_REDUCE_SUM, s);
          if (st != 0) throw std::runtime_error("mixed-out sponge: reduce callback failed");
        }
        hipLaunchKernelGGL((k_mixed_out_finish<C, PH>), dim3(1), dim3(1), 0, s, prm_k, op->d_forcing, z);
        HIP_CHECK(hipGetLastError());
      }
    }
    const int grid = static_cast<int>((op->ndofs + 255) / 256);
    hipLaunchKernelGGL((k_forcing<C, PH>), dim3(grid), dim3(256), 0, s, m, prm_k, op->d_forcing, x, op->d_gradUp, y);
    HIP_CHECK(hipGetLastError());
  };
  if (op->timing) {
    op->ev = op->evs[op->sets_recorded % tpsrhs_operator::MAXSETS];
    HIP_CHECK(hipEventRecord(op->ev[0], s));
  }
  const MeshDev all = op->mesh_dev();
  if (op->sweep_alt) op->sweep_parity ^= 1;
  if (op->topo.num_shared == 0) {
    traces(all, nblocks);
    if (op->timing) HIP_CHECK(hipEventRecord(op->ev[1], s));
    gradient(all, nblocks);
    if (op->timing) HIP_CHECK(hipEventRecord(op->ev[2], s));
    if (gradients_only) return;
    nr_update(all);
    flux(all, nblocks);
  } else {
    if (!op->d_blocks_halo) {
      std::vector<int> halo, interior;
      std::vector<char> is_halo(nblocks, 0);
      for (int i = 0; i < op->topo.num_shared; i++) is_halo[(op->topo.shared_slot[i] / op->nfaces) / C::EPB] = 1;
      for (int b = 0; b < nblocks; b++) (is_halo[b] ? halo : interior).push_back(b);
      op->n_blocks_halo = static_cast<int>(halo.size());
      op->n_blocks_interior = static_cast<int>(interior.size());
      op->d_blocks_halo = dev_upload(halo);
      op->d_blocks_interior = dev_upload(interior);
      HIP_CHECK(hipStreamCreateWithFlags(&op->comm_stream, hipStreamNonBlocking));
      for (auto &e : op->ev_halo) HIP_CHECK(hipEventCreateWithFlags(&e, hipEventDisableTiming));
    }
    MeshDev mh = all, mi = all;
    mh.blocks = op->d_blocks_halo;
    mi.blocks = op->d_blocks_interior;
    const int nh = op->n_blocks_halo, ni = op->n_blocks_interior;
    hipStream_t c = op->comm_stream;
    traces(mh, nh);
    HIP_CHECK(hipEventRecord(op->ev_halo[0], s));
    if (ni) traces(mi, ni);
    if (op->timing) HIP_CHECK(hipEventRecord(op->ev[1], s));
    if (ni) gradient(mi, ni);
    HIP_CHECK(hipStreamWaitEvent(c, op->ev_halo[0], 0));
    exchange(op, 0, op->d_TA, 2 * PH::NEQ, C::NF, c);
    HIP_CHECK(hipEventRecord(op->ev_halo[1], c));
    HIP_CHECK(hipStreamWaitEvent(s, op->ev_halo[1], 0));
    gradient(mh, nh);
    if (op->timing) HIP_CHECK(hipEventRecord(op->ev[2], s));
    if (gradients_only) return;
    HIP_CHECK(hipEventRecord(op->ev_halo[2], s));
    nr_update(all);
    if (ni) flux(mi, ni);
    HIP_CHECK(hipStreamWaitEvent(c, op->ev_halo[2], 0));
    exchange(op, 1, op->d_TB, PH::NEQ - 1, C::NQ, c);
    HIP_CHECK(hipEventRecord(op->ev_halo[3], c));
    HIP_CHECK(hipStreamWaitEvent(s, op->ev_halo[3], 0));
    flux(mh, nh);
  }
  forcing(all);
  if constexpr (PH::HAS_NR_BC) {
    if (op->n_nr_faces > 0) {
      op->bstate_cur = 1 - op->bstate_cur;
      op->bstate_init = true;
    }
  }
  if (op->timing) {
    HIP_CHECK(hipEventRecord(op->ev[3], s));
    op->sets_recorded++;
  }
}

template <class PH>
void launch_point_eval(tpsrhs_operator *op, int quantity, int64_t n, const double *U, double *out) {
  const int grid = static_cast<int>((n + 255) / 256);
  if (grid == 0) return;
  hipLaunchKernelGGL((k_point_eval<PH>), dim3(grid), dim3(256), 0, op->stream, kernel_params<PH>(op), quantity, n, U, out);
  HIP_CHECK(hipGetLastError());
}

inline void upload_tables(int dim, int order, int nc = 0) {
  const Tables1D tabs = make_tables(order, dim, nc, nc);
  const size_t off = ((static_cast<size_t>(nc) * 2 + (dim - 2)) * (TPSRHS_MAXORDER + 1) + order) * sizeof(Tables1D);
  HIP_CHECK(hipMemcpyToSymbol(HIP_SYMBOL(c_tab), &tabs, sizeof(Tables1D), off, hipMemcpyHostToDevice));
}

template <int DIM, class PH>
void pick_order_nc(tpsrhs_operator *op) {
  upload_tables(DIM, op->order, 1);
  op->point_eval = &launch_point_eval<PH>;
  if constexpr (PH::AXISYM) {
    throw Unsupported("the Gauss-Lobatto pair is built for the planar 2-D and the 3-D formulation");
  } else {
    switch (op->order) {
// ... 37 lines not shown
```

### tps_amd/csrc/physics_plasma.hpp

```cpp
#ifndef TPSRHS_PHYSICS_PLASMA_HPP_
#define TPSRHS_PHYSICS_PLASMA_HPP_

#include <hip/hip_runtime.h>

#include "physics_dryair.hpp"

namespace tpsrhs {

#pragma clang fp reciprocal(on)

constexpr double kRgas = 8.3144598;
constexpr double kAvogadro = 6.0221409e+23;
constexpr double kBoltz = kRgas / kAvogadro;
constexpr double kEps0 = 8.8541878128e-12;
constexpr double kQe = 1.60218e-19;
constexpr double kMolarQe = kQe * kAvogadro;
constexpr double kPi = 3.14159265358979323846;
constexpr double kXeps = 1.0e-30;

struct TableDev {
  int n, x_log, f_log, pad;
  const double *x, *a, *b;
  double x0, inv_dx;
};
// ... 120 lines not shown
      {0.0683, 1.9774, 1.2033, 0.8264}, {0.0346, 4.5177, 1.2132, 0.9294}},
     {{0, 0, 0, 0}, {0.4128, 1.2436, 1.1830, 1.0123}, {0.2203, 1.8832, 1.2059, 0.9851}, {0.1323, 2.7248, 1.2129, 0.9847},
      {0, 0, 0, 0}}}};
__device__ inline double ArAr11(double lnT) { return 2.2910e-18 * fexp(-0.3032 * lnT); }
__device__ inline double ArAr22(double T) { return 1.7e-18 * fast_rsqrt(fast_sqrt(T)); }
__device__ inline double iArAr22(double sqrtT) { return fast_sqrt(sqrtT) * (1.0 / 1.7e-18); }
__device__ inline double ArAr1P11(double lnT) { return 4.574321e-18 * fexp(-0.1805 * lnT); }
__device__ inline double eAr1r(int r, double logT) {
  const double C[5][9] = {
      {6.36254140e-18, 1.84835040e-18, -5.87727093e-18, 3.20023027e-18, -8.50509054e-19, 1.28163820e-19,
       -1.11712910e-20, 5.25649382e-22, -1.03296658e-23},
      {1.91338172e-17, 5.45418129e-18, -1.78361685e-17, 9.75657946e-18, -2.61115722e-18, 3.98310268e-19,
       -3.53503678e-20, 1.70375066e-21, -3.45211955e-23},
      {3.04685398e-17, 8.39750994e-18, -2.88132528e-17, 1.60147037e-17, -4.34837891e-18, 6.73136845e-19,
       -6.06704580e-20, 2.97216168e-21, -6.12760944e-23},
      {3.90777949e-17, 1.04696956e-17, -3.73774204e-17, 2.10610498e-17, -5.79029566e-18, 9.07573157e-19,
       -8.28466766e-20, 4.11188110e-21, -8.59225098e-23},
      {4.41333290e-17, 1.15696010e-17, -4.25651305e-17, 2.42442440e-17, -6.73359258e-18, 1.06641697e-18,
       -9.83933863e-20, 4.93775812e-21, -1.04362372e-22}};
  double fit = C[r - 1][0] * fast_rcp(logT), pw = 1.0;
#pragma unroll
  for (int k = 1; k < 9; k++) {
    fit += C[r - 1][k] * pw;
    pw *= logT;
  }
  return fit;
}
template <int NR>
__device__ inline void eAr1r_n(double logT, double (&fit)[NR]) {
  static_assert(NR <= 5, "five fits");
  constexpr double C[5][9] = {
      {6.36254140e-18, 1.84835040e-18, -5.87727093e-18, 3.20023027e-18, -8.50509054e-19, 1.28163820e-19,
       -1.11712910e-20, 5.25649382e-22, -1.03296658e-23},
      {1.91338172e-17, 5.45418129e-18, -1.78361685e-17, 9.75657946e-18, -2.61115722e-18, 3.98310268e-19,
       -3.53503678e-20, 1.70375066e-21, -3.45211955e-23},
      {3.04685398e-17, 8.39750994e-18, -2.88132528e-17, 1.60147037e-17, -4.34837891e-18, 6.73136845e-19,
       -6.06704580e-20, 2.97216168e-21, -6.12760944e-23},
      {3.90777949e-17, 1.04696956e-17, -3.73774204e-17, 2.10610498e-17, -5.79029566e-18, 9.07573157e-19,
       -8.28466766e-20, 4.11188110e-21, -8.59225098e-23},
      {4.41333290e-17, 1.15696010e-17, -4.25651305e-17, 2.42442440e-17, -6.73359258e-18, 1.06641697e-18,
       -9.83933863e-20, 4.93775812e-21, -1.04362372e-22}};
  const double il = fast_rcp(logT);
#pragma unroll
  for (int r = 0; r < NR; r++) fit[r] = C[r][0] * il;
  double pw = 1.0;
#pragma unroll
  for (int k = 1; k < 9; k++) {
#pragma unroll
    for (int r = 0; r < NR; r++) fit[r] += C[r][k] * pw;
    pw *= logT;
  }
}
}

#ifndef TPSRHS_PLASMA_MINW_FLUX
#define TPSRHS_PLASMA_MINW_FLUX 2
#endif
#ifndef TPSRHS_PLASMA_MINW_GRAD3
#define TPSRHS_PLASMA_MINW_GRAD3 2
#endif
#ifndef TPSRHS_PLASMA_MINW_GRAD_LEAN
#define TPSRHS_PLASMA_MINW_GRAD_LEAN 3
#endif
enum { TRANSPORT_CONSTANT = 0, TRANSPORT_ARGON_MINIMAL = 1, TRANSPORT_ARGON_MIXTURE = 2 };

template <int DIM_, int NVEL_, int NSP_, bool AMBI, bool TWOT, int TRANSPORT>
struct PlasmaPhys {
  static constexpr int DIM = DIM_, NVEL = NVEL_, NSP = NSP_;
  static constexpr int NACTIVE = AMBI ? NSP_ - 2 : NSP_ - 1;
  static constexpr int NEQ = NVEL_ + 2 + NACTIVE + (TWOT ? 1 : 0);
  static constexpr int IE = NSP_ - 2, IB = NSP_ - 1;
  static constexpr int ITH = NVEL_ + 1, ITE = NEQ - 1;
  static constexpr bool HAS_SOURCE = true;
  static constexpr bool TWO_TEMPERATURE = TWOT;
  static constexpr int MAX_ORDER = 4;
  static constexpr bool HAS_NR_BC = false;
  static constexpr bool LES = false;
  static constexpr bool HAS_MIXED_OUT = false;
  static constexpr bool VISC_USES_GRAD_RHO = true;
  static constexpr bool AXISYM = NVEL_ > DIM_;
  static constexpr int MINW_GRAD = (NSP_ > 3) ? 1 : TPSRHS_PLASMA_MINW_GRAD3;
  static constexpr bool LEAN_TRACE = (NSP_ == 3) && (DIM_ == 3);
  static constexpr bool LEAN_ONE_HEX = LEAN_TRACE && !TWOT && TRANSPORT == TRANSPORT_ARGON_MINIMAL;
  static constexpr bool LAUNDER_FLUX = false;
  static constexpr int minw_grad(int dim, int p, int nc) {
    return (LEAN_TRACE && dim == 3 && !nc && p <= 3) ? TPSRHS_PLASMA_MINW_GRAD_LEAN : MINW_GRAD;
  }
  static constexpr int MINW_FLUX = (NSP_ > 6 || (NSP_ > 3 && DIM_ == 3)) ? 1 : TPSRHS_PLASMA_MINW_FLUX;
  typedef PlasmaParams<NSP_> Params;
  typedef const Params *KArg;
  typedef const Params __attribute__((address_space(4))) &PRef;
  typedef const BcDev __attribute__((address_space(4))) &BcRef;
  __device__ static inline PRef pref(KArg k) { return *(const Params __attribute__((address_space(4))) *)k; }
  __device__ static inline PRef relaunder(PRef p) {
    const unsigned long long a = reinterpret_cast<unsigned long long>(&p);
    unsigned lo = __builtin_amdgcn_readfirstlane(static_cast<unsigned>(a));
    unsigned hi = __builtin_amdgcn_readfirstlane(static_cast<unsigned>(a >> 32));
    asm volatile("" : "+s"(lo), "+s"(hi));
    return *reinterpret_cast<const Params __attribute__((address_space(4))) *>((static_cast<unsigned long long>(hi) << 32) | lo);
  }
  struct Transport {};

  struct State {
    double ir, k, p, pe, Th, Te, c;
    double vel[NVEL];
    double n[NSP];
  };

  __device__ static inline void number_densities(PRef p, const double *U, double *n) {
#pragma unroll
    for (int sp = 0; sp < NSP; sp++) n[sp] = 0.0;
#pragma unroll
    for (int sp = 0; sp < NACTIVE; sp++) n[sp] = U[NVEL + 2 + sp] * p.imw[sp];
    double rhoB = U[0];
#pragma unroll
    for (int sp = 0; sp < NACTIVE; sp++) rhoB -= p.mw[sp] * n[sp];
    if (AMBI) {
      double ne = 0.0;
#pragma unroll
      for (int sp = 0; sp < NACTIVE; sp++) ne += p.charge[sp] * n[sp];
      ne = fmax(ne, 0.0);
      n[IE] = ne;
      rhoB -= ne * p.mw[IE];
    }
    n[IB] = rhoB * p.imw[IB];
  }
  __device__ static inline double heavies_cv(PRef p, const double *n) {
    double c = 0.0;
#pragma unroll
    for (int sp = 0; sp < NACTIVE; sp++)
      if (sp != IE) c += n[sp] * p.cv[sp];
    return c + n[IB] * p.cv[IB];
  }
  __device__ static inline double heavies_n(const double *n) {
    double nh = 0.0;
#pragma unroll
    for (int sp = 0; sp < NACTIVE; sp++)
      if (sp != IE) nh += n[sp];
    return nh + n[IB];
  }
  __device__ static inline State make_state(PRef p, const double *U) {
    State s;
    number_densities(p, U, s.n);
    s.ir = fast_rcp(U[0]);
    double m2 = 0.0;
#pragma unroll
    for (int d = 0; d < NVEL; d++) {
      m2 += U[1 + d] * U[1 + d];
      s.vel[d] = U[1 + d] * s.ir;
    }
    s.k = m2 * s.ir;
    const double chv = heavies_cv(p, s.n);
    double ctot = chv;
    if (!TWOT) ctot += s.n[IE] * p.cv[IE];
    double e = U[ITH];
#pragma unroll
    for (int sp = 0; sp < NSP - 2; sp++) e -= s.n[sp] * p.eform[sp];
    double Th = -0.5 * s.k + e;
    if (TWOT) Th -= U[ITE];
    s.Th = Th * fast_rcp(ctot);
    s.Te = TWOT ? U[ITE] * fast_rcp(s.n[IE] * p.cv[IE]) : s.Th;
    const double nh = heavies_n(s.n);
    s.pe = s.n[IE] * kRgas * s.Te;
    s.p = kRgas * (nh * s.Th + s.n[IE] * s.Te);
    const double gamma = 1.0 + nh * kRgas * fast_rcp(chv);
    s.c = fast_sqrt(gamma * s.p * s.ir);
// ... 1272 lines not shown
```

### tps_amd/csrc/plasma_family.hpp

```cpp
#ifndef TPSRHS_PLASMA_FAMILY_HPP_
#define TPSRHS_PLASMA_FAMILY_HPP_

#include "operator.hpp"
#include "physics_plasma.hpp"

template <int DIM, int NVEL, int NSP, bool AMBI, bool TWOT, int TR>
static void pick_plasma_orders(tpsrhs_operator *op) {
  typedef PlasmaPhys<DIM, NVEL, NSP, AMBI, TWOT, TR> PH;
  if (op->nc) {
#ifndef TPSRHS_PLASMA_HIGH_ORDERS
    if constexpr (NVEL == DIM) {
      pick_order_nc<DIM, PH>(op);
      return;
    } else
#endif
    {
      throw Unsupported("Gauss-Lobatto basis + rule: planar 2-D and 3-D, polynomial orders 1..3");
    }
  }
  upload_tables(DIM, op->order);
  op->point_eval = &launch_point_eval<PH>;
  switch (op->order) {
#ifndef TPSRHS_PLASMA_HIGH_ORDERS
    case 1: op->launch = &launch_all<DIM, 1, PH>; break;
    case 2: op->launch = &launch_all<DIM, 2, PH>; break;
    case 3: op->launch = &launch_all<DIM, 3, PH>; break;
#else
    case 4: op->launch = &launch_all<DIM, 4, PH>; break;
    case 5: op->launch = &launch_all<DIM, 5, PH>; break;
#endif
    default: throw Unsupported("plasma kernels of this family: polynomial order " + std::to_string(op->order) + " is not built");
  }
}

template <int DIM, int NVEL, int NSP, bool AMBI>
static void pick_plasma_family(tpsrhs_operator *op, bool two_temperature, int transport) {
  if (transport == TRANSPORT_CONSTANT) {
    if (two_temperature)
      pick_plasma_orders<DIM, NVEL, NSP, AMBI, true, TRANSPORT_CONSTANT>(op);
    else
      pick_plasma_orders<DIM, NVEL, NSP, AMBI, false, TRANSPORT_CONSTANT>(op);
  } else if (transport == TRANSPORT_ARGON_MIXTURE) {
    if constexpr (NSP <= 7) {
      if (two_temperature)
        pick_plasma_orders<DIM, NVEL, NSP, AMBI, true, TRANSPORT_ARGON_MIXTURE>(op);
      else
        pick_plasma_orders<DIM, NVEL, NSP, AMBI, false, TRANSPORT_ARGON_MIXTURE>(op);
    } else {
      throw Unsupported("argon_mixture transport supports at most 7 species");
    }
  } else {
    if constexpr (NSP == 3) {
      if (two_temperature)
        pick_plasma_orders<DIM, NVEL, NSP, AMBI, true, TRANSPORT_ARGON_MINIMAL>(op);
      else
        pick_plasma_orders<DIM, NVEL, NSP, AMBI, false, TRANSPORT_ARGON_MINIMAL>(op);
    } else {
      throw Unsupported("argon_minimal transport is the ternary (Ar, Ar.+1, E) model");
    }
  }
}

#if TPSRHS_STAMP
extern "C" int tpsrhs_debug_stamps(unsigned int *out, int nblocks) {
  const size_t bytes = static_cast<size_t>(nblocks) * tpsrhs::NSTAMP * sizeof(unsigned int);
  return hipMemcpyFromSymbol(out, HIP_SYMBOL(tpsrhs::g_stamp), bytes) == hipSuccess ? 0 : 1;
}
#endif

#if TPSRHS_DUMPF
extern "C" int tpsrhs_debug_dumpf(double *out, int n) {
  return hipMemcpyFromSymbol(out, HIP_SYMBOL(tpsrhs::g_dumpf), static_cast<size_t>(n) * sizeof(double)) == hipSuccess ? 0 : 1;
}
#endif

#define TPSRHS_PLASMA_FAMILY(name, DIM, NVEL, NSP, AMBI)                                                              \
  extern "C" int name(tpsrhs_operator *op, int two_temperature, int transport, char *err, int errlen) {               \
    auto say = [&](const char *what) {                                                                                \
      if (err && errlen > 0) {                                                                                        \
        std::strncpy(err, what, static_cast<size_t>(errlen) - 1);                                                     \
        err[errlen - 1] = 0;                                                                                          \
      }                                                                                                               \
    };                                                                                                                \
    try {                                                                                                             \
      pick_plasma_family<DIM, NVEL, NSP, AMBI>(op, two_temperature != 0, transport);                                  \
      return TPSRHS_OK;                                                                                               \
    } catch (const Unsupported &e) {                                                                                  \
      say(e.what());                                                                                                  \
      return TPSRHS_ERR_UNSUPPORTED;                                                                                  \
    } catch (const DeviceError &e) {                                                                                  \
      say(e.what());                                                                                                  \
      return TPSRHS_ERR_DEVICE;                                                                                       \
    } catch (const std::invalid_argument &e) {                                                                        \
      say(e.what());                                                                                                  \
      return TPSRHS_ERR_INVALID_ARGUMENT;                                                                             \
    } catch (const std::exception &e) {                                                                               \
      say(e.what());                                                                                                  \
      return TPSRHS_ERR_DEVICE;                                                                                       \
    }                                                                                                                 \
  }
#endif
```

### tps_amd/csrc/tpsrhs.hip

```cpp
#include "operator.hpp"
#include "physics_dryair.hpp"
#include "physics_dryair_axisym.hpp"
#include "physics_plasma.hpp"
#include "plasma_params_host.hpp"

#include <dlfcn.h>

#include <cmath>
#include <map>
#include <mutex>
#include <new>
#include <thread>

void pick_dryair_axisym(tpsrhs_operator *op);
void pick_lte_axisym(tpsrhs_operator *op);
void pick_dryair_les(tpsrhs_operator *op);

static thread_local std::string g_last_error;

namespace {

typedef int (*family_pick_fn)(tpsrhs_operator *, int, int, char *, int);
family_pick_fn load_family(const std::string &unit) {
  static std::mutex mu;
  static std::map<std::string, family_pick_fn> loaded;
  std::lock_guard<std::mutex> lock(mu);
  auto it = loaded.find(unit);
  if (it != loaded.end()) return it->second;
  std::vector<std::string> dirs;
  if (const char *env = std::getenv("TPSRHS_FAMILY_PATH")) {
    std::string e(env);
    size_t pos = 0;
    while (pos <= e.size()) {
      const size_t c = e.find(':', pos);
      const std::string d = e.substr(pos, c == std::string::npos ? std::string::npos : c - pos);
      if (!d.empty()) dirs.push_back(d);
      if (c == std::string::npos) break;
      pos = c + 1;
    }
  }
  Dl_info info;
  if (dladdr(reinterpret_cast<const void *>(&load_family), &info) && info.dli_fname) {
    const std::string self(info.dli_fname);
    const size_t slash = self.rfind('/');
    dirs.push_back(slash == std::string::npos ? std::string(".") : self.substr(0, slash));
  }
  std::string tried;
  for (const std::string &d : dirs) {
    const std::string path = d + "/libtpsrhs_" + unit + ".so";
    if (void *h = dlopen(path.c_str(), RTLD_NOW | RTLD_LOCAL)) {
      const std::string sym = "pick_" + unit;
      auto fn = reinterpret_cast<family_pick_fn>(dlsym(h, sym.c_str()));
      if (!fn) throw std::runtime_error(path + " does not export " + sym);
      loaded[unit] = fn;
      return fn;
    }
    const char *why = dlerror();
    tried += "\n  " + path + ": " + (why ? why : "not loadable");
  }
  throw Unsupported("kernel family " + unit + " is not available (run __graft_entry__.build()):" + tried);
}

TableDev upload_table(tpsrhs_operator *op, const tpsrhs_table &t) {
  std::vector<double> buf;
  TableDev td = table_coeffs(t, buf);
  double *d = dev_upload(buf);
  op->d_extra.push_back(d);
  td.x = d;
  td.a = d + td.n;
  td.b = d + 2 * td.n;
  return td;
}

template <int NSP>
void fill_plasma_params(tpsrhs_operator *op, const tpsrhs_disc *disc, const tpsrhs_physics *phys, int num_bcs,
                        const tpsrhs_bc *bcs) {
  static_assert(sizeof(PlasmaParams<NSP>) <= sizeof(op->params), "parameter block too large");
  PlasmaParams<NSP> &p = *new (op->params) PlasmaParams<NSP>;
  std::unique_ptr<ChemDev> c(new ChemDev);
  try {
    tpsrhs::fill_plasma_params<NSP>(p, *c, disc, phys, num_bcs, bcs, [op](const tpsrhs_table &t) { return upload_table(op, t); });
  } catch (const UnsupportedConfig &e) {
    throw Unsupported(e.what());
  }
  ChemDev *dc = dev_alloc<ChemDev>(1);
  HIP_CHECK(hipMemcpy(dc, c.get(), sizeof(ChemDev), hipMemcpyHostToDevice));
  op->d_chem = dc;
  p.chem = dc;
}

std::vector<double> element_sizes(const std::vector<double> &verts, int dim, int ne) {
  std::vector<double> h(ne);
  const int nv = 1 << dim;
  for (int e = 0; e < ne; e++) {
    const double *V = &verts[static_cast<size_t>(e) * nv * dim];
    double J[3][3] = {{0, 0, 0}, {0, 0, 0}, {0, 0, 0}};
    for (int v = 0; v < nv; v++)
      for (int a = 0; a < dim; a++) {
        const double sgn = ((v >> a) & 1) ? 1.0 : -1.0;
        for (int i = 0; i < dim; i++) J[i][a] += sgn * V[v * dim + i] / (nv / 2);
      }
    double A[3][3];
    for (int a = 0; a < dim; a++)
      for (int b = 0; b < dim; b++) {
        double t = 0.0;
        for (int i = 0; i < dim; i++) t += J[i][a] * J[i][b];
        A[a][b] = t;
      }
    for (int sweep = 0; sweep < 30; sweep++) {
      double off = 0.0;
      for (int a = 0; a < dim; a++)
        for (int b = a + 1; b < dim; b++) off += A[a][b] * A[a][b];
      if (off == 0.0) break;
      for (int a = 0; a < dim; a++)
        for (int b = a + 1; b < dim; b++) {
          if (A[a][b] == 0.0) continue;
          const double theta = (A[b][b] - A[a][a]) / (2.0 * A[a][b]);
          const double t = (theta >= 0.0 ? 1.0 : -1.0) / (std::fabs(theta) + std::sqrt(theta * theta + 1.0));
          const double c = 1.0 / std::sqrt(t * t + 1.0), sn = t * c;
          for (int k = 0; k < dim; k++) {
            const double aka = A[k][a], akb = A[k][b];
            A[k][a] = c * aka - sn * akb;
            A[k][b] = sn * aka + c * akb;
          }
          for (int k = 0; k < dim; k++) {
            const double aak = A[a][k], abk = A[b][k];
            A[a][k] = c * aak - sn * abk;
            A[b][k] = sn * aak + c * abk;
          }
        }
    }
    double lmin = A[0][0];
    for (int a = 1; a < dim; a++) lmin = std::min(lmin, A[a][a]);
    h[e] = std::sqrt(std::max(lmin, 0.0));
  }
  return h;
// ... 277 lines not shown
        lp->ehint = dh;
        lp->nhint = nh;
        lp->e0 = ex[0];
        lp->inv_de = 1.0 / de;
      }
      auto same_grid = [](const tpsrhs_table &a, const tpsrhs_table &b) {
        if (a.n_data != b.n_data || a.x_log_scale != b.x_log_scale) return 0;
        for (int k = 0; k < a.n_data; k++)
          if (a.x_data[k] != b.x_data[k]) return 0;
        return 1;
      };
      lp->thermo_same_grid = same_grid(in.energy_table, in.gas_constant_table) && same_grid(in.energy_table, in.sound_speed_table);
      lp->trans_same_grid = same_grid(in.viscosity_table, in.conductivity_table);
      lp->tab_mu = upload_table(op, in.viscosity_table);
      lp->tab_k = upload_table(op, in.conductivity_table);
      lp->tab_sigma = upload_table(op, in.electric_conductivity_table);
      lp->radiation = phys->radiation.model;
      if (lp->radiation == TPSRHS_NET_EMISSION) lp->tab_nec = upload_table(op, phys->radiation.nec_table);
    }
    d.gamma = phys->dry_air.specific_heat_ratio;
    d.Rg = phys->dry_air.gas_constant;
    d.inv_Rg = 1.0 / d.Rg;
    d.visc_mult = phys->dry_air.visc_mult;
    d.bulk_mult = phys->dry_air.bulk_visc_mult;
    d.C1 = phys->dry_air.sutherland_C1;
    d.S0 = phys->dry_air.sutherland_S0;
    d.cp_div_pr = d.gamma * d.Rg / (phys->dry_air.sutherland_Pr * (d.gamma - 1.0));
    d.eq_system = phys->eq_system;
    d.use_bc_in_grad = disc->use_bc_in_grad;
    d.use_roe = disc->use_roe ? 1 : 0;
    d.ref_length = disc->ref_length > 0.0 ? disc->ref_length : 1.0;
    d.num_bcs = num_bcs;
    for (int i = 0; i < num_bcs; i++) {
      d.bc[i].category = bcs[i].category;
      d.bc[i].type = bcs[i].type;
      for (int k = 0; k < 4 + TPSRHS_MAXSPECIES; k++) d.bc[i].data[k] = bcs[i].data[k];
    }
    bool any_nr = false;
    for (int i = 0; i < num_bcs; i++) any_nr = any_nr || is_non_reflecting(bcs[i].category, bcs[i].type);
    const bool les = !heavy2d && (phys->sgs.model_type != TPSRHS_SGS_NONE || phys->visc_sponge.enabled);
    if (les) {
      if (phys->sgs.model_type < 0 || phys->sgs.model_type > TPSRHS_SGS_SIGMA)
        throw std::invalid_argument("unknown sgs.model_type");
      if (disc->axisymmetric || op->nc || any_nr)
        throw Unsupported("sub-grid scale model / viscous sponge: built for dry air, planar 2-D and 3-D, Gauss-Legendre pair, "
                          "reflecting boundary types");
      if (phys->sgs.model_type != TPSRHS_SGS_NONE && op->dim != 3)
        throw Unsupported("sub-grid scale models need dim == 3 (the reference's strain tensor indexes three directions)");
      if (phys->visc_sponge.enabled && !(phys->visc_sponge.width > 0.0))
        throw std::invalid_argument("visc_sponge.width must be positive");
      d.sgs_type = phys->sgs.model_type;
      d.sgs_const = phys->sgs.model_const > 0.0 ? phys->sgs.model_const
                                                : (d.sgs_type == TPSRHS_SGS_SMAGORINSKY ? 0.12 : (d.sgs_type == TPSRHS_SGS_SIGMA ? 0.135 : 0.0));
      d.sgs_floor = phys->sgs.model_floor;
      d.vs_enabled = phys->visc_sponge.enabled ? 1 : 0;
      double nmag = 0.0;
      for (int k = 0; k < op->dim; k++) nmag += phys->visc_sponge.normal[k] * phys->visc_sponge.normal[k];
      nmag = std::sqrt(nmag);
      if (phys->visc_sponge.enabled && !(nmag > 0.0)) throw std::invalid_argument("visc_sponge.normal is zero");
      for (int k = 0; k < 3; k++) {
        d.vs_n[k] = (k < op->dim && nmag > 0.0) ? phys->visc_sponge.normal[k] / nmag : 0.0;
        d.vs_p[k] = (k < op->dim) ? phys->visc_sponge.point[k] : 0.0;
      }
      d.vs_width = phys->visc_sponge.enabled ? phys->visc_sponge.width : 1.0;
      d.vs_ratio = phys->visc_sponge.enabled ? phys->visc_sponge.ratio : 1.0;
      std::vector<double> delta = mesh->elem_size ? std::vector<double>(mesh->elem_size, mesh->elem_size + tp.ne)
                                                  : element_sizes(tp.verts, op->dim, tp.ne);
      for (double &v : delta) v /= op->order;
      double *dd = dev_upload(delta);
      op->d_extra.push_back(dd);
      d.elem_delta = dd;
      pick_dryair_les(op);
    } else if (lte)
      pick_lte_axisym(op);
    else if (disc->axisymmetric)
      pick_dryair_axisym(op);
    else if (op->dim == 3)
      any_nr ? pick_order<3, DryAirPhys<3, true>>(op) : pick_order<3, DryAirPhys<3>>(op);
    else
      any_nr ? pick_order<2, DryAirPhys<2, true>>(op) : pick_order<2, DryAirPhys<2>>(op);
  }

  op->d_verts = dev_upload(tp.verts);
  if (op->nc) op->d_minv = dev_upload(inverse_mass_matrices(tp.verts, op->dim, op->order, op->ne));
  {
    std::vector<int2> fi(tp.face_nbr.size());
    for (size_t i = 0; i < fi.size(); i++) fi[i] = make_int2(tp.face_nbr[i], tp.face_orient[i]);
    op->d_face_info = dev_upload(fi);
  }
  if (!plasma && !disc->axisymmetric) {
    std::vector<int2> nrf;
    std::vector<int> ordinal(tp.face_nbr.size(), -1);
    bool any_nr = false;
    for (int i = 0; i < num_bcs; i++) any_nr = any_nr || is_non_reflecting(bcs[i].category, bcs[i].type);
    if (any_nr) {
      DryAirParams &d = *reinterpret_cast<DryAirParams *>(op->params);
      for (size_t slot = 0; slot < tp.face_nbr.size(); slot++) {
        const int nb = tp.face_nbr[slot];
        if (nb >= 0) continue;
        const int b = -nb - 1;
        if (!is_non_reflecting(bcs[b].category, bcs[b].type)) continue;
        ordinal[slot] = static_cast<int>(nrf.size());
        nrf.push_back(make_int2(static_cast<int>(slot), b));
        double *t1 = &d.bc[b].data[4];
        if (t1[0] == 0.0 && t1[1] == 0.0 && t1[2] == 0.0) {
          const int e = static_cast<int>(slot) / op->nfaces, lf = static_cast<int>(slot) % op->nfaces, D = lf >> 1, sd = lf & 1;
          const int nv = 1 << op->dim, a = (op->dim == 2) ? 1 - D : (D == 0 ? 1 : 0);
          const int c0 = sd << D, c1 = c0 | (1 << a);
          double mod = 0.0, t[3] = {0, 0, 0};
          for (int k = 0; k < op->dim; k++) {
            t[k] = tp.verts[(static_cast<size_t>(e) * nv + c1) * op->dim + k] - tp.verts[(static_cast<size_t>(e) * nv + c0) * op->dim + k];
            mod += t[k] * t[k];
          }
          for (int k = 0; k < 3; k++) t1[k] = t[k] / std::sqrt(mod);
        }
      }
      if (tp.num_shared > 0 && !op->reduce)
        throw std::runtime_error("halo: a partitioned mesh with non-reflecting patches needs runtime.reduce");
      op->n_nr_faces = static_cast<int>(nrf.size());
      op->d_bc_sums = dev_alloc<double>(MAXBC * (TPSRHS_MAXEQUATIONS + 1));
      HIP_CHECK(hipMemset(op->d_bc_sums, 0, MAXBC * (TPSRHS_MAXEQUATIONS + 1) * sizeof(double)));
      if (!nrf.empty()) {
        op->d_nr_faces = dev_upload(nrf);
        op->d_nr_ordinal = dev_upload(ordinal);
        const size_t n = nrf.size() * static_cast<size_t>(op->nq) * op->neq;
        for (int k = 0; k < 2; k++) {
          op->d_bstate[k] = dev_alloc<double>(n);
          HIP_CHECK(hipMemset(op->d_bstate[k], 0, n * sizeof(double)));
        }
      }
    }
    op->has_nr = any_nr;
  }
  if (op->ndofs >= (int64_t(1) << 31)) throw Unsupported("more than 2^31 nodes per rank");
  const int64_t nslots = static_cast<int64_t>(op->ne) * op->nfaces + tp.num_shared;
  op->d_Up = dev_alloc<double>(op->neq * op->ndofs);
  op->d_gradUp = dev_alloc<double>(op->dim * op->neq * op->ndofs);
  op->d_TA = dev_alloc<double>(nslots * 2 * op->neq * op->nf);
  op->d_TB = dev_alloc<double>(nslots * (op->neq - 1) * op->nq);
  HIP_CHECK(hipMemset(op->d_TA, 0, nslots * 2 * op->neq * op->nf * sizeof(double)));
  HIP_CHECK(hipMemset(op->d_TB, 0, nslots * (op->neq - 1) * op->nq * sizeof(double)));
  op->d_speed = dev_alloc<double>(1);
  HIP_CHECK(hipMemset(op->d_speed, 0, sizeof(double)));
  if (tp.num_shared > 0) {
    op->d_shared_slot = dev_upload(tp.shared_slot);
    op->d_shared_orient = dev_upload(tp.shared_orient);
    const int64_t per0 = 2 * op->neq * op->nf, per1 = static_cast<int64_t>(op->neq - 1) * op->nq;
    op->d_send = dev_alloc<double>(tp.num_shared * std::max(per0, per1));
    for (size_t i = 0; i < tp.nbr_offsets.size(); i++) {
      op->send_off[0].push_back(tp.nbr_offsets[i] * per0);
      op->send_off[1].push_back(tp.nbr_offsets[i] * per1);
    }
    op->recv_off[0] = op->send_off[0];
    op->recv_off[1] = op->send_off[1];
  }
  for (auto &set : op->evs)
    for (auto &e : set) HIP_CHECK(hipEventCreate(&e));
}

int fail(int code, const std::string &msg) {
  g_last_error = msg;
  return code;
}

template <class F>
int guarded(F &&f) {
// ... 372 lines not shown
          d.msum = ds;
          for (int eq = 0; eq < TPSRHS_MAXEQUATIONS; eq++) d.target[eq] = 0.0;
        } else {
          if (s.solution_type != TPSRHS_SPONGE_USERDEF) throw std::invalid_argument("tpsrhs_set_forcing: unknown sponge solution type");
          for (int eq = 0; eq < TPSRHS_MAXEQUATIONS; eq++) d.target[eq] = eq < h->neq ? s.target_U[eq] : 0.0;
          if (!(d.target[0] > 0.0)) throw std::invalid_argument("tpsrhs_set_forcing: sponge target density must be positive");
        }
      }
    }
    const ForcingDev prev = h->forcing;
    const bool prev_active = h->forcing_active;
    h->forcing = f;
    try {
      upload_forcing(h);
      HIP_CHECK(hipStreamSynchronize(h->stream));
    } catch (...) {
      h->forcing = prev;
      h->forcing_active = prev_active;
      throw;
    }
    std::vector<void *> old;
    old.swap(h->d_mixed_out);
    h->d_mixed_out = fresh;
    guard.keep = true;
    h->config_epoch++;
    for (void *q : old) (void)hipFree(q);
  });
}

int tpsrhs_set_mixing_length(tpsrhs_handle h, const double *distance, const tpsrhs_mixing_length *in) {
  if (!h) return fail(TPSRHS_ERR_INVALID_ARGUMENT, "tpsrhs_set_mixing_length: NULL handle");
  return guarded([&] {
    if (distance) {
      if (!in) throw std::invalid_argument("tpsrhs_set_mixing_length: parameters missing");
      const bool plasma = h->phys.working_fluid == TPSRHS_USER_DEFINED;
      if (h->dim != 2 || !(plasma || h->nvel == 3))
        throw Unsupported("mixing-length model: built for the 2-D kernels (mixtures planar / axisymmetric, dry air axisymmetric)");
      if (h->nc) throw Unsupported("mixing-length model: Gauss-Legendre pair");
      if (!(in->max_mixing_length >= 0.0)) throw std::invalid_argument("tpsrhs_set_mixing_length: negative max_mixing_length");
      h->mixlen.distance = distance;
      h->mixlen.lmax = in->max_mixing_length;
      h->mixlen.prt = in->pr_ratio;
      h->mixlen.bulk = in->bulk_multiplier;
    } else {
      h->mixlen.distance = nullptr;
    }
    h->config_epoch++;
  });
}

int tpsrhs_set_joule_heating(tpsrhs_handle h, const double *joule_heating) {
  if (!h) return fail(TPSRHS_ERR_INVALID_ARGUMENT, "tpsrhs_set_joule_heating: NULL handle");
  return guarded([&] {
    if (joule_heating && h->nvel != 3) throw Unsupported("JouleHeating needs three velocity components (3-D or axisymmetric)");
    h->forcing.joule = joule_heating;
    h->config_epoch++;
    upload_forcing(h);
  });
}

int tpsrhs_update_gradients(tpsrhs_handle h, const double *x) {
  if (!h || !x) return fail(TPSRHS_ERR_INVALID_ARGUMENT, "tpsrhs_update_gradients: NULL argument");
  return guarded([&] {
    HIP_CHECK(hipSetDevice(h->device));
    h->launch(h, x, nullptr, true);
  });
}

int tpsrhs_get_primitives(tpsrhs_handle h, double *up_out) {
  if (!h || !up_out) return fail(TPSRHS_ERR_INVALID_ARGUMENT, "tpsrhs_get_primitives: NULL argument");
  return guarded([&] {
    HIP_CHECK(hipMemcpyAsync(up_out, h->d_Up, sizeof(double) * h->neq * h->ndofs, hipMemcpyDeviceToDevice, h->stream));
  });
}

int tpsrhs_get_gradients(tpsrhs_handle h, double *gradup_out) {
  if (!h || !gradup_out) return fail(TPSRHS_ERR_INVALID_ARGUMENT, "tpsrhs_get_gradients: NULL argument");
  return guarded([&] {
    HIP_CHECK(hipMemcpyAsync(gradup_out, h->d_gradUp, sizeof(double) * h->dim * h->neq * h->ndofs,
                             hipMemcpyDeviceToDevice, h->stream));
  });
}

int64_t tpsrhs_height(tpsrhs_handle h) { return h ? h->neq * h->ndofs : -1; }
int64_t tpsrhs_num_dofs(tpsrhs_handle h) { return h ? h->ndofs : -1; }
int tpsrhs_num_equation(tpsrhs_handle h) { return h ? h->neq : -1; }

int tpsrhs_enable_kernel_timing(tpsrhs_handle h, int enable) {
  if (!h) return TPSRHS_ERR_INVALID_ARGUMENT;
  h->timing = enable != 0;
  h->sets_recorded = 0;
  return TPSRHS_OK;
}

int tpsrhs_kernel_times(tpsrhs_handle h, int capacity, const char **names, double *milliseconds) {
  if (!h || h->sets_recorded == 0) return 0;
  if (hipStreamSynchronize(h->stream) != hipSuccess) return 0;
  const int nsets = static_cast<int>(std::min<int64_t>(h->sets_recorded, tpsrhs_operator::MAXSETS));
  int n = 0;
  for (int k = 0; k < NKERN && n < capacity; k++, n++) {
    double sum = 0.0;
    for (int i = 0; i < nsets; i++) {
      float ms = 0.f;
      if (hipEventElapsedTime(&ms, h->evs[i][k], h->evs[i][k + 1]) != hipSuccess) return n;
      sum += ms;
    }
    if (names) names[n] = kKernelNames[k];
    if (milliseconds) milliseconds[n] = sum / nsets;
  }
  return n;
}

int tpsrhs_eval_pointwise(tpsrhs_handle h, int quantity, int64_t n, const double *U, double *out) {
  if (!h || n < 0 || !U || !out || quantity < 0 || quantity > 3) return fail(TPSRHS_ERR_INVALID_ARGUMENT, "eval_pointwise");
  return guarded([&] {
    HIP_CHECK(hipSetDevice(h->device));
    h->point_eval(h, quantity, n, U, out);
    HIP_CHECK(hipStreamSynchronize(h->stream));
  });
}

namespace {
__global__ void k_table_eval(TableDev t, int64_t n, const double *__restrict__ x, double *__restrict__ f) {
  const int64_t i = static_cast<int64_t>(blockIdx.x) * 256 + threadIdx.x;
  if (i < n) f[i] = table_eval(t, x[i]);
}
}

namespace {
__global__ void k_math_eval(int fn, int64_t n, const double *__restrict__ x, double *__restrict__ y) {
  const int64_t i = static_cast<int64_t>(blockIdx.x) * 256 + threadIdx.x;
  if (i >= n) return;
  const double v = x[i];
  double r;
  switch (fn) {
    case 0: r = fexp(v); break;
    case 1: r = fexp<false>(v); break;
    case 2: r = flog(v); break;
    case 3: r = flog_pos(v); break;
    case 4: r = fast_rcp(v); break;
    case 5: r = fast_sqrt(v); break;
    default: r = fast_rsqrt(v); break;
  }
  y[i] = r;
}
}

int tpsrhs_math_eval(int function, int64_t n, const double *x, double *y) {
  if (function < 0 || function > 6 || n < 0 || !x || !y) return fail(TPSRHS_ERR_INVALID_ARGUMENT, "math_eval");
  return guarded([&] {
    int ndev = 0;
    if (hipGetDeviceCount(&ndev) != hipSuccess || ndev == 0) throw std::runtime_error("no HIP device visible");
    if (n > 0) {
      hipLaunchKernelGGL(k_math_eval, dim3(static_cast<unsigned>((n + 255) / 256)), dim3(256), 0, nullptr, function, n, x, y);
      HIP_CHECK(hipGetLastError());
    }
    HIP_CHECK(hipDeviceSynchronize());
  });
}

int tpsrhs_table_eval(const tpsrhs_table *table, int64_t n, const double *x, double *f) {
  if (!table || n < 0 || !x || !f) return fail(TPSRHS_ERR_INVALID_ARGUMENT, "table_eval");
  return guarded([&] {
    int ndev = 0;
    if (hipGetDeviceCount(&ndev) != hipSuccess || ndev == 0) throw std::runtime_error("no HIP device visible");
    tpsrhs_operator tmp;
// ... 82 lines not shown
```

### tps_amd/rhs_operator.py

```python
from __future__ import annotations

import ctypes as C

import numpy as np
import torch

from . import capi


class TpsRhsError(RuntimeError):
    def __init__(self, status, where):
        lib = capi.load()
        self.status = status
        msg = lib.tpsrhs_last_error().decode()
        super().__init__(f"{where}: {lib.tpsrhs_status_string(status).decode()}: {msg}")


class RHSoperator:

    def __init__(self, host_mesh, disc, physics, bcs=(), device=0, halo=None, stream=None):
        self._lib = capi.load()
        if not torch.cuda.is_available():
            raise RuntimeError("tps_amd.RHSoperator needs a HIP device (torch.cuda.is_available() is False)")
        self.device = torch.device("cuda", device)
        self._margs = capi.MeshArgs(host_mesh)
        self._disc, self._physics = disc, physics
        self._bcs = (capi.BC * max(1, len(bcs)))(*bcs)
        rt = capi.Runtime()
        rt.device = device
        st = stream if stream is not None else torch.cuda.current_stream(self.device)
        self._stream = st
        rt.stream = C.c_void_p(st.cuda_stream)
        self._halo = halo
        if halo is not None and hasattr(halo, "c_halo"):
            rt.halo, rt.halo_ctx = halo.c_halo, halo.ctx
            rt.reduce, rt.reduce_ctx = halo.c_reduce, halo.ctx
        elif halo is not None:
            self._halo_cb = capi.HALO_FN(halo.callback)
            rt.halo = self._halo_cb
            if hasattr(halo, "reduce_callback"):
                self._reduce_cb = capi.REDUCE_FN(halo.reduce_callback)
                rt.reduce = self._reduce_cb
        self._rt = rt
        h = C.c_void_p()
        st_code = self._lib.tpsrhs_create(C.byref(self._margs.c), C.byref(disc), C.byref(physics), len(bcs),
                                          self._bcs, C.byref(rt), C.byref(h))
        if st_code != 0:
            raise TpsRhsError(st_code, "tpsrhs_create")
        self._h = h
        self.dim = host_mesh.dim
        self.num_equation = int(self._lib.tpsrhs_num_equation(h))
        self.NDofs = int(self._lib.tpsrhs_num_dofs(h))
        self.max_char_speed = 0.0
        self._time = 0.0

    def Height(self) -> int:
        return int(self._lib.tpsrhs_height(self._h))

    def SetTime(self, t: float):
        self._time = float(t)

    def GetTime(self) -> float:
        return self._time

    def Mult(self, x: torch.Tensor, y: torch.Tensor, want_max_char_speed: bool = False):
        self._check(x)
        self._check(y)
        mcs = C.c_double(0.0)
        st = self._lib.tpsrhs_mult(self._h, C.c_void_p(x.data_ptr()), C.c_void_p(y.data_ptr()), self._time,
                                   C.byref(mcs) if want_max_char_speed else None)
        if st != 0:
            raise TpsRhsError(st, "tpsrhs_mult")
        if want_max_char_speed:
            self.max_char_speed = mcs.value

    def updateGradients(self, x: torch.Tensor):
        self._check(x)
        st = self._lib.tpsrhs_update_gradients(self._h, C.c_void_p(x.data_ptr()))
        if st != 0:
            raise TpsRhsError(st, "tpsrhs_update_gradients")

    def getPrimitives(self) -> torch.Tensor:
        out = torch.empty(self.num_equation * self.NDofs, dtype=torch.float64, device=self.device)
        st = self._lib.tpsrhs_get_primitives(self._h, C.c_void_p(out.data_ptr()))
        if st != 0:
            raise TpsRhsError(st, "tpsrhs_get_primitives")
        return out.view(self.num_equation, self.NDofs)

    def getGradients(self) -> torch.Tensor:
        out = torch.empty(self.dim * self.num_equation * self.NDofs, dtype=torch.float64, device=self.device)
        st = self._lib.tpsrhs_get_gradients(self._h, C.c_void_p(out.data_ptr()))
        if st != 0:
            raise TpsRhsError(st, "tpsrhs_get_gradients")
        return out.view(self.dim, self.num_equation, self.NDofs)

    def getPlasmaConductivity(self, x: torch.Tensor) -> torch.Tensor:
        self._check(x)
        out = torch.empty(self.NDofs, dtype=torch.float64, device=self.device)
        st = self._lib.tpsrhs_get_plasma_conductivity(self._h, C.c_void_p(x.data_ptr()), C.c_void_p(out.data_ptr()))
        if st != 0:
            raise TpsRhsError(st, "tpsrhs_get_plasma_conductivity")
        return out

    def enable_kernel_timing(self, on=True):
        self._lib.tpsrhs_enable_kernel_timing(self._h, 1 if on else 0)

    def kernel_times(self):
        names = (C.c_char_p * 8)()
        ms = (C.c_double * 8)()
        n = self._lib.tpsrhs_kernel_times(self._h, 8, names, ms)
        return {names[i].decode(): ms[i] for i in range(n)}

    def mult_times(self):
        ms = (C.c_double * 128)()
        n = self._lib.tpsrhs_mult_times(self._h, 128, ms)
        return [ms[i] for i in range(n)]

    def rk4_step(self, x: torch.Tensor, time: float, dt: float, want_max_char_speed=False, want_nan_count=False):
        self._check(x)
        t = C.c_double(time)
        speed = C.c_double(0.0)
        bad = C.c_int64(0)
        st = self._lib.tpsrhs_rk4_step(self._h, C.c_void_p(x.data_ptr()), C.byref(t), float(dt),
                                       C.byref(speed) if want_max_char_speed else None,
                                       C.byref(bad) if want_nan_count else None)
        if st != 0:
            raise RuntimeError(f"tpsrhs_rk4_step: {capi.STATUS.get(st, st)}: {self._lib.tpsrhs_last_error().decode()}")
        if want_max_char_speed:
            self.max_char_speed = speed.value
        if want_nan_count:
            self.nan_count = bad.value
        return t.value

    def advance(self, x: torch.Tensor, time: float, dt: float, num_steps: int, constant_dt=True, cfl=0.0, hmin=0.0):
        self._check(x)
        t, d, bad = C.c_double(time), C.c_double(dt), C.c_int64(0)
        st = self._lib.tpsrhs_advance(self._h, C.c_void_p(x.data_ptr()), C.byref(t), C.byref(d), int(num_steps),
                                      1 if constant_dt else 0, float(cfl), float(hmin), C.byref(bad))
        if st != 0:
            raise TpsRhsError(st, "tpsrhs_advance")
        return t.value, d.value, bad.value

    def setDt(self, dt: float):
        st = self._lib.tpsrhs_set_dt(self._h, float(dt))
        if st != 0:
            raise TpsRhsError(st, "tpsrhs_set_dt")

    def setForcing(self, forcing):
        st = self._lib.tpsrhs_set_forcing(self._h, C.byref(forcing) if forcing is not None else None)
        if st != 0:
            raise TpsRhsError(st, "tpsrhs_set_forcing")

    def setJouleHeating(self, joule_heating):
        if joule_heating is not None:
            if (joule_heating.dtype != torch.float64 or not joule_heating.is_cuda or not joule_heating.is_contiguous()
                    or joule_heating.numel() != self.NDofs):
                raise ValueError("expected a contiguous float64 CUDA tensor of NDofs entries")
        self._joule = joule_heating
        st = self._lib.tpsrhs_set_joule_heating(
            self._h, C.c_void_p(joule_heating.data_ptr()) if joule_heating is not None else None)
        if st != 0:
            raise TpsRhsError(st, "tpsrhs_set_joule_heating")

    def setMixingLength(self, distance, max_mixing_length=0.0, pr_ratio=1.0, lewis=1.0, bulk_multiplier=0.0):
        if distance is not None:
            if (distance.dtype != torch.float64 or not distance.is_cuda or not distance.is_contiguous()
                    or distance.numel() != self.NDofs):
                raise ValueError("expected a contiguous float64 CUDA tensor of NDofs entries")
        self._distance = distance
        prm = capi.MixingLength(float(max_mixing_length), float(pr_ratio), float(lewis), float(bulk_multiplier))
        st = self._lib.tpsrhs_set_mixing_length(self._h, C.c_void_p(distance.data_ptr()) if distance is not None else None,
                                                C.byref(prm))
        if st != 0:
            raise TpsRhsError(st, "tpsrhs_set_mixing_length")

    def kernel_bytes(self):
        names = (C.c_char_p * 8)()
        b = (C.c_double * 8)()
# ... 46 lines not shown
```

Measured before the change: 12720.

## Precompute per-element face normals, jump normals and nodal adjugates into a stored geometry table

```diff
diff --git a/include/tpsrhs.h b/include/tpsrhs.h
--- a/include/tpsrhs.h
+++ b/include/tpsrhs.h
@@ -254,6 +254,7 @@
 
 int tpsrhs_get_primitives(tpsrhs_handle h, double *up_out);
 int tpsrhs_get_gradients(tpsrhs_handle h, double *gradup_out);
+int64_t tpsrhs_geometry_table(tpsrhs_handle h, double *host_out, int64_t capacity, int *layout);
 int tpsrhs_get_plasma_conductivity(tpsrhs_handle h, const double *x, double *sigma_out);
 
 enum tpsrhs_point_quantity {
diff --git a/tps_amd/capi.py b/tps_amd/capi.py
--- a/tps_amd/capi.py
+++ b/tps_amd/capi.py
@@ -558,6 +558,8 @@
     lib.tpsrhs_update_gradients.argtypes = [vp, vp]
     lib.tpsrhs_get_primitives.argtypes = [vp, vp]
     lib.tpsrhs_get_gradients.argtypes = [vp, vp]
+    lib.tpsrhs_geometry_table.restype = C.c_int64
+    lib.tpsrhs_geometry_table.argtypes = [vp, vp, C.c_int64, vp]
     lib.tpsrhs_get_plasma_conductivity.argtypes = [vp, vp, vp]
     lib.tpsrhs_height.restype = C.c_int64
     lib.tpsrhs_height.argtypes = [vp]
@@ -590,7 +592,7 @@
 
 EXPORTED_SYMBOLS = [
     "tpsrhs_create", "tpsrhs_destroy", "tpsrhs_mult", "tpsrhs_mult_host", "tpsrhs_update_gradients",
-    "tpsrhs_get_primitives", "tpsrhs_get_gradients", "tpsrhs_get_plasma_conductivity", "tpsrhs_height", "tpsrhs_num_dofs", "tpsrhs_num_equation",
+    "tpsrhs_get_primitives", "tpsrhs_get_gradients", "tpsrhs_geometry_table", "tpsrhs_get_plasma_conductivity", "tpsrhs_height", "tpsrhs_num_dofs", "tpsrhs_num_equation",
     "tpsrhs_enable_kernel_timing", "tpsrhs_kernel_times", "tpsrhs_mult_times", "tpsrhs_kernel_bytes",
     "tpsrhs_eval_pointwise", "tpsrhs_table_eval", "tpsrhs_math_eval", "tpsrhs_face_tables",
     "tpsrhs_rk4_step", "tpsrhs_advance", "tpsrhs_set_dt", "tpsrhs_set_forcing", "tpsrhs_set_joule_heating", "tpsrhs_set_mixing_length", "tpsrhs_status_string",
diff --git a/tps_amd/csrc/kernels.hpp b/tps_amd/csrc/kernels.hpp
--- a/tps_amd/csrc/kernels.hpp
+++ b/tps_amd/csrc/kernels.hpp
@@ -30,6 +30,15 @@
 #endif
 #ifndef TPSRHS_LEAN_GENERAL
 #define TPSRHS_LEAN_GENERAL 0
+#endif
+#ifndef TPSRHS_GEOM_FACE
+#define TPSRHS_GEOM_FACE 1
+#endif
+#ifndef TPSRHS_GEOM_JUMP
+#define TPSRHS_GEOM_JUMP 1
+#endif
+#ifndef TPSRHS_GEOM_NODE
+#define TPSRHS_GEOM_NODE 1
 #endif
 constexpr int cmax(int a, int b) { return a > b ? a : b; }
 
@@ -202,10 +211,34 @@
   int64_t ndofs;
   const double *verts;
   const int2 *face_info;
-  const double *minv;
+  union {
+    const double *minv;
+    const double *geom;
+  };
   MixLenDev ml;
   VsDev vs;
 };
+template <class PH, class = void>
+struct stored_geom_trait {
+  static constexpr bool value = false;
+};
+template <class PH>
+struct stored_geom_trait<PH, std::enable_if_t<PH::STORED_GEOM || !PH::STORED_GEOM>> {
+  static constexpr bool value = PH::STORED_GEOM;
+};
+template <class C, class PH>
+struct GeomTab {
+  static constexpr bool SHAPE = stored_geom_trait<PH>::value && C::DIM == 3 && !C::NC && C::EPB == 1 && C::BLOCK == 64 && C::TQ <= C::BLOCK;
+  static constexpr bool FACE = SHAPE && TPSRHS_GEOM_FACE, JUMP = SHAPE && TPSRHS_GEOM_JUMP, NODE = SHAPE && TPSRHS_GEOM_NODE;
+  static constexpr bool ON = FACE || JUMP || NODE;
+  static constexpr int N_FACE = FACE ? 3 * 3 * C::BLOCK : 0, N_JUMP = JUMP ? 6 * 3 * C::NF : 0, N_NODE = NODE ? 10 * C::NPE : 0;
+  static constexpr int O_FACE = 0, O_JUMP = N_FACE, O_NODE = N_FACE + N_JUMP, STRIDE = N_FACE + N_JUMP + N_NODE;
+};
+template <class C, class PH>
+__device__ inline const double *geom_of(const MeshDev &m, int e) {
+  return m.geom + static_cast<int64_t>(e) * GeomTab<C, PH>::STRIDE;
+}
+
 __device__ inline EddyCtx closure_ctx(const MeshDev &m, bool dist_on, double dist, const double *X, double *park) {
   EddyCtx ec = dist_on ? eddy_at(m.ml, dist) : eddy_off();
   if (m.vs.enabled) {
@@ -1084,10 +1117,18 @@
   else
     face_normal_at<C, (C::DIM == 3 ? 2 : 0)>(V, s, ta, tb, n);
 }
+template <class C, class PH, int D>
+__device__ inline void issue_jump_normals(const MeshDev &m, int e, const int *idx, double *jn) {
+  typedef GeomTab<C, PH> G;
+  const int fn = idx[tan_a<C>(D)] + C::N1 * idx[tan_b<C>(D)];
+  const double *gj = geom_of<C, PH>(m, e) + G::O_JUMP + (2 * D) * C::DIM * C::NF + fn;
+#pragma unroll
+  for (int k = 0; k < 2 * C::DIM; k++) jn[k] = gj[k * C::NF];
+}
 template <class C, class PH>
 __device__ inline void grad_jump_nodal(int D, const int2 *sFI, typename PH::PRef prm, const double *Town,
                                        const double *Tnb, const double *sV, const Tab<C> &tab, int le_n, const int *idx,
-                                       double inv_mass, double *g) {
+                                       double inv_mass, double *g, const double *jn = nullptr) {
   constexpr int NEQ = PH::NEQ, DIM = C::DIM;
   const int da = (DIM == 2) ? 1 - D : (D == 0 ? 1 : 0), db = (D == 2) ? 1 : 2;
   const int ia = idx[da], ib = (DIM == 3) ? idx[db] : 0;
@@ -1105,7 +1146,12 @@
     }
     if (nb < 0 && prm.use_bc_in_grad) PH::bc_grad_prim(prm, prm.bc[-nb - 1], u1, u2);
     double n[DIM];
-    face_normal_rt<C>(D, &sV[le_n * C::NV * DIM], s, tab.x[ia], (DIM == 3) ? tab.x[ib] : 0.0, n);
+    if constexpr (GeomTab<C, PH>::JUMP) {
+#pragma unroll
+      for (int i = 0; i < DIM; i++) n[i] = s ? jn[DIM + i] : jn[i];
+    } else {
+      face_normal_rt<C>(D, &sV[le_n * C::NV * DIM], s, tab.x[ia], (DIM == 3) ? tab.x[ib] : 0.0, n);
+    }
     const double c = 0.5 * wf * inv_mass * (s ? tab.b1[idx[D]] : tab.b0[idx[D]]);
 #pragma unroll
     for (int dd = 0; dd < DIM; dd++) {
@@ -1435,7 +1481,13 @@
     if (on) {
       double wq, Xq[DIM];
       nb = sFI[le * C::NFACES + 2 * d + s].x;
-      face_geometry_rt<C>(d, &sV[le * C::NV * DIM], tab, s, q, n, wq, Xq);
+      if constexpr (GeomTab<C, PH>::FACE) {
+        const double *gf = geom_of<C, PH>(m, e0 + le) + GeomTab<C, PH>::O_FACE + d * (DIM * C::BLOCK) + tid;
+#pragma unroll
+        for (int i = 0; i < DIM; i++) n[i] = gf[i * C::BLOCK];
+      } else {
+        face_geometry_rt<C>(d, &sV[le * C::NV * DIM], tab, s, q, n, wq, Xq);
+      }
     }
     const int np_lane = on ? PH::visc_passes(prm, nb) : 0;
     const int npass = (__ballot(np_lane == 2) != 0) ? 2 : ((__ballot(np_lane >= 1) != 0) ? 1 : 0);
@@ -1673,7 +1725,13 @@
     if (on) {
       double wq, Xq[DIM];
       nb = sFI[le * C::NFACES + 2 * d + s].x;
-      face_geometry_rt<C>(d, &sV[le * C::NV * DIM], tab, s, q, n, wq, Xq);
+      if constexpr (GeomTab<C, PH>::FACE) {
+        const double *gf = geom_of<C, PH>(m, e0 + le) + GeomTab<C, PH>::O_FACE + d * (DIM * C::BLOCK) + tid;
+#pragma unroll
+        for (int i = 0; i < DIM; i++) n[i] = gf[i * C::BLOCK];
+      } else {
+        face_geometry_rt<C>(d, &sV[le * C::NV * DIM], tab, s, q, n, wq, Xq);
+      }
     }
     const int np_lane = on ? PH::visc_passes(prm, nb) : 0;
     const int npass = (__ballot(np_lane == 2) != 0) ? 2 : ((__ballot(np_lane >= 1) != 0) ? 1 : 0);
@@ -1832,6 +1890,58 @@
 }
 
 template <class C, class PH>
+__global__ __launch_bounds__(C::BLOCK) void k_geometry(MeshDev m, double *__restrict__ geom) {
+  typedef GeomTab<C, PH> G;
+  constexpr int DIM = C::DIM;
+  static_assert(G::ON, "stored geometry: 3-D collocated one-hex blocks of a physics that asks for it");
+  const Tables1D &ct = c_tab[C::NC][DIM - 2][C::P];
+  __shared__ Tab<C> tab;
+  __shared__ double sV[C::EPB * C::NV * DIM];
+  const int tid = threadIdx.x;
+  const int e0 = static_cast<int>(blockIdx.x);
+  if (e0 >= m.ne) return;
+  load_tables<C>(tab, ct);
+  load_vertices<C>(sV, m, e0);
+  block_sync<C::BLOCK>();
+  double *out = geom + static_cast<int64_t>(e0) * G::STRIDE;
+  if constexpr (G::FACE) {
+#pragma clang loop unroll(disable)
+    for (int d = 0; d < DIM; d++) {
+      double n[DIM] = {0.0, 0.0, 0.0};
+      if (tid < C::TQ) {
+        const int pf = tid / C::NQ, q = tid - pf * C::NQ;
+        double wq, Xq[DIM];
+        face_geometry_rt<C>(d, sV, tab, pf & 1, q, n, wq, Xq);
+      }
+#pragma unroll
+      for (int i = 0; i < DIM; i++) out[G::O_FACE + (d * DIM + i) * C::BLOCK + tid] = n[i];
+    }
+  }
+  if constexpr (G::JUMP) {
+    for (int item = tid; item < C::NFACES * C::NF; item += C::BLOCK) {
+      const int f = item / C::NF, fn = item - f * C::NF;
+      double n[DIM];
+      face_normal_rt<C>(f >> 1, sV, f & 1, tab.x[fn % C::N1], tab.x[fn / C::N1], n);
+#pragma unroll
+      for (int i = 0; i < DIM; i++) out[G::O_JUMP + (f * DIM + i) * C::NF + fn] = n[i];
+    }
+  }
+  if constexpr (G::NODE) {
+    if (tid < C::NPE) {
+      const int idx[3] = {tid % C::N1, (tid / C::N1) % C::N1, tid / (C::N1 * C::N1)};
+      double xi[DIM], J[DIM * DIM], A[DIM * DIM];
+#pragma unroll
+      for (int d = 0; d < DIM; d++) xi[d] = tab.x[idx[d]];
+      jacobian<DIM>(sV, xi, J);
+      const double det = adjugate<DIM>(J, A);
+#pragma unroll
+      for (int k = 0; k < DIM * DIM; k++) out[G::O_NODE + k * C::NPE + tid] = A[k];
+      out[G::O_NODE + DIM * DIM * C::NPE + tid] = det;
+    }
+  }
+}
+
+template <class C, class PH>
 __global__ __launch_bounds__(C::BLOCK, (C::NC && PH::HEAVY) ? 1 : PH::minw_grad(C::DIM, C::P, C::NC)) void k_gradient(MeshDev m, typename PH::KArg prm_k,
                                                        const double *__restrict__ U, const double *__restrict__ TA,
                                                        double *__restrict__ Upout, double *__restrict__ gradUp,
@@ -1897,6 +2007,11 @@
 #pragma unroll
   for (int k = 0; k < NEQ * DIM; k++) g[k] = 0.0;
   double inv_mass = 0.0;
+  typedef GeomTab<C, PH> G;
+  double jn0[G::JUMP ? 2 * DIM : 1], jn1[G::JUMP ? 2 * DIM : 1], jn2[G::JUMP ? 2 * DIM : 1];
+  if constexpr (G::JUMP) {
+    if (node_on) issue_jump_normals<C, PH, 0>(m, e0 + le_n, idx, jn0);
+  }
   if constexpr (C::NC) {
     nc_volume_gradient<C, NEQ>(sUp, pool + L::O_V, sV, tab, ct, node_on, le_n, nd, tid, g);
   } else if (node_on) {
@@ -1907,8 +2022,16 @@
       xi[d] = tab.x[idx[d]];
       iwn *= tab.iw[idx[d]];
     }
-    jacobian<DIM>(&sV[le_n * C::NV * DIM], xi, J);
-    const double det = adjugate<DIM>(J, A);
+    double det;
+    if constexpr (G::NODE) {
+      const double *gn = geom_of<C, PH>(m, e0 + le_n) + G::O_NODE + nd;
+#pragma unroll
+      for (int k = 0; k < DIM * DIM; k++) A[k] = gn[k * C::NPE];
+      det = gn[DIM * DIM * C::NPE];
+    } else {
+      jacobian<DIM>(&sV[le_n * C::NV * DIM], xi, J);
+      det = adjugate<DIM>(J, A);
+    }
     const double idet = fast_rcp(det);
     inv_mass = iwn * idet;
     double Dr[DIM][C::N1];
@@ -1946,7 +2069,9 @@
       if constexpr (C::NC) {
         nc_grad_jump<C, PH, D>(sFI, prm, sJ, pool + L::O_V, sV, tab, ct, node_on, le_n, idx, tid, g);
       } else {
-        if (node_on) grad_jump_nodal<C, PH>(D, sFI, prm, sJ, sJ + NEQ * C::TN, sV, tab, le_n, idx, inv_mass, g);
+        if (node_on)
+          grad_jump_nodal<C, PH>(D, sFI, prm, sJ, sJ + NEQ * C::TN, sV, tab, le_n, idx, inv_mass, g,
+                                 G::JUMP ? (D == 0 ? jn0 : (D == 1 ? jn1 : jn2)) : nullptr);
         block_sync<C::BLOCK>();
       }
     };
@@ -1955,12 +2080,18 @@
     block_sync<C::BLOCK>();
     store_neighbour_traces<C, NEQ>(ta0, sJ, sJ + NEQ * C::TN, tid);
     block_sync<C::BLOCK>();
+    if constexpr (G::JUMP) {
+      if (node_on) issue_jump_normals<C, PH, 1>(m, e0 + le_n, idx, jn1);
+    }
     jump(std::integral_constant<int, 0>());
     if (LATE && DIM == 3) issue_neighbour_traces<C, (DIM == 3 ? 2 : 0), NEQ>(sFI, TA, 2 * NEQ * C::NF, NEQ, ta2, tid);
     trace_lines<C, 1, NEQ>(sUp, sJ, ct, tid);
     block_sync<C::BLOCK>();
     store_neighbour_traces<C, NEQ>(ta1, sJ, sJ + NEQ * C::TN, tid);
     block_sync<C::BLOCK>();
+    if constexpr (G::JUMP) {
+      if (node_on) issue_jump_normals<C, PH, (DIM == 3 ? 2 : 0)>(m, e0 + le_n, idx, jn2);
+    }
     jump(std::integral_constant<int, 1>());
     if (DIM == 3) {
       trace_lines<C, (DIM == 3 ? 2 : 0), NEQ>(sUp, sJ, ct, tid);
@@ -2383,6 +2514,14 @@
                                      const NbTraces<C, PH::NEQ> &ta, const NbFlux<C, PH::NEQ> &tb, bool node_on,
                                      int le_n, const int *idx, double *z, int tid) {
   constexpr int NEQ = PH::NEQ, DIM = C::DIM;
+  double ng[GeomTab<C, PH>::FACE ? DIM : 1];
+  if constexpr (GeomTab<C, PH>::FACE) {
+    if (tid < C::TQ && tb.nb[0] != INT32_MIN) {
+      const double *gf = geom_of<C, PH>(m, e0) + GeomTab<C, PH>::O_FACE + D * (DIM * C::BLOCK) + tid;
+#pragma unroll
+      for (int i = 0; i < DIM; i++) ng[i] = gf[i * C::BLOCK];
+    }
+  }
   trace_lines<C, D, NEQ>(sU, X, ct, tid);
   block_sync<C::BLOCK>();
   store_neighbour_traces<C, NEQ>(ta, X, X + NEQ * C::TN, tid);
@@ -2411,7 +2550,13 @@
     }
     PH::clamp_species(u1);
     double n[DIM], wq, Xq[DIM];
-    face_geometry<C, D>(&sV[le * C::NV * DIM], tab, s, q, n, wq, Xq);
+    if constexpr (GeomTab<C, PH>::FACE) {
+#pragma unroll
+      for (int i = 0; i < DIM; i++) n[i] = ng[i];
+      wq = tab.wq[q % C::Q1] * tab.wq[q / C::Q1];
+    } else {
+      face_geometry<C, D>(&sV[le * C::NV * DIM], tab, s, q, n, wq, Xq);
+    }
     if (TPSRHS_ABLATE & 4) {
 #pragma unroll
       for (int eq = 0; eq < NEQ; eq++) fh[rd][eq] = u1[eq] + u2[eq] * n[0];
@@ -2628,6 +2773,14 @@
   double src[NEQ];
 #pragma unroll
   for (int eq = 0; eq < NEQ; eq++) src[eq] = 0.0;
+  double gnode[GeomTab<C, PH>::NODE ? DIM * DIM + 1 : 1];
+  if constexpr (GeomTab<C, PH>::NODE) {
+    if (node_on) {
+      const double *gn = geom_of<C, PH>(m, e0 + le_n) + GeomTab<C, PH>::O_NODE + nd;
+#pragma unroll
+      for (int k = 0; k < DIM * DIM + 1; k++) gnode[k] = gn[k * C::NPE];
+    }
+  }
   if (node_on) {
     double F[NEQ * DIM];
     double radius = 1.0;
@@ -2700,8 +2853,15 @@
       wn *= tab.w[idx[d]];
       iwn *= tab.iw[idx[d]];
     }
-    jacobian<DIM>(&sV[le_n * C::NV * DIM], xi, J);
-    const double det = adjugate<DIM>(J, A);
+    double det;
+    if constexpr (GeomTab<C, PH>::NODE) {
+#pragma unroll
+      for (int k = 0; k < DIM * DIM; k++) A[k] = gnode[k];
+      det = gnode[DIM * DIM];
+    } else {
+      jacobian<DIM>(&sV[le_n * C::NV * DIM], xi, J);
+      det = adjugate<DIM>(J, A);
+    }
     inv_mass = iwn * fast_rcp(det);
     if (PH::AXISYM) {
       inv_mass *= fast_rcp(radius);
diff --git a/tps_amd/csrc/operator.hpp b/tps_amd/csrc/operator.hpp
--- a/tps_amd/csrc/operator.hpp
+++ b/tps_amd/csrc/operator.hpp
@@ -60,6 +60,14 @@
 const char *kKernelNames[NKERN] = {"k_traces", "k_gradient", "k_flux"};
 
 }
+
+constexpr int TPSRHS_LAYOUT_VERSION = 6;
+struct LayoutStamp {
+  int version;
+  unsigned op_bytes, rk_bytes, mesh_bytes;
+};
+struct tpsrhs_operator;
+inline LayoutStamp layout_stamp();
 
 struct tpsrhs_operator {
   int dim = 0, order = 0, neq = 0, nvel = 0;
@@ -137,6 +145,9 @@
   bool sweep_alt = true;
   int sweep_parity = 0;
   VsDev vs2d = {};
+  double *d_geom = nullptr;
+  int geom_layout[8] = {};
+  void (*build_geom)(tpsrhs_operator *) = nullptr;
 
   MeshDev mesh_dev() const {
     MeshDev m;
@@ -162,6 +173,7 @@
     if (d_chem) (void)hipFree(d_chem);
     if (d_params) (void)hipFree(d_params);
     if (d_minv) (void)hipFree(d_minv);
+    if (d_geom) (void)hipFree(d_geom);
     if (d_TA2) (void)hipFree(d_TA2);
     if (d_rk) (void)hipFree(d_rk);
     if (d_nan) (void)hipFree(d_nan);
@@ -183,6 +195,11 @@
   }
 };
 
+inline LayoutStamp layout_stamp() {
+  return {TPSRHS_LAYOUT_VERSION, static_cast<unsigned>(sizeof(tpsrhs_operator)), static_cast<unsigned>(sizeof(RkDev)),
+          static_cast<unsigned>(sizeof(MeshDev))};
+}
+
 namespace {
 
 template <class PH>
@@ -215,6 +232,26 @@
   const int st = op->halo(op->halo_ctx, phase, op->d_send, recv, static_cast<int>(tp.nbr_ranks.size()),
                           tp.nbr_ranks.data(), op->send_off[phase].data(), op->recv_off[phase].data(), stream);
   if (st != 0) throw std::runtime_error("halo callback failed in phase " + std::to_string(phase));
+}
+
+template <int DIM, int P, class PH, int NC = 0>
+void build_geometry(tpsrhs_operator *op) {
+  typedef Cfg<DIM, P, NC> C;
+  typedef GeomTab<C, PH> G;
+  if constexpr (G::ON) {
+    if (op->d_geom) {
+      (void)hipFree(op->d_geom);
+      op->d_geom = nullptr;
+    }
+    op->d_geom = dev_alloc<double>(static_cast<size_t>(op->ne) * G::STRIDE);
+    const int layout[8] = {G::STRIDE, G::O_FACE, G::N_FACE, G::O_JUMP, G::N_JUMP, G::O_NODE, G::N_NODE, 0};
+    std::memcpy(op->geom_layout, layout, sizeof layout);
+    if (op->ne > 0) {
+      hipLaunchKernelGGL((k_geometry<C, PH>), dim3(op->ne), dim3(C::BLOCK), 0, op->stream, op->mesh_dev(), op->d_geom);
+      HIP_CHECK(hipGetLastError());
+      HIP_CHECK(hipStreamSynchronize(op->stream));
+    }
+  }
 }
 
 template <int DIM, int P, class PH, int NC = 0>
@@ -314,7 +351,11 @@
     op->ev = op->evs[op->sets_recorded % tpsrhs_operator::MAXSETS];
     HIP_CHECK(hipEventRecord(op->ev[0], s));
   }
-  const MeshDev all = op->mesh_dev();
+  MeshDev all = op->mesh_dev();
+  if constexpr (GeomTab<C, PH>::ON) {
+    if (!op->d_geom) throw DeviceError("stored geometry: the operator has no table (tpsrhs_operator::build_geom was not run)");
+    all.geom = op->d_geom;
+  }
   if (op->sweep_alt) op->sweep_parity ^= 1;
   if (op->topo.num_shared == 0) {
     traces(all, nblocks);
diff --git a/tps_amd/csrc/physics_plasma.hpp b/tps_amd/csrc/physics_plasma.hpp
--- a/tps_amd/csrc/physics_plasma.hpp
+++ b/tps_amd/csrc/physics_plasma.hpp
@@ -226,6 +226,7 @@
   static constexpr int MINW_GRAD = (NSP_ > 3) ? 1 : TPSRHS_PLASMA_MINW_GRAD3;
   static constexpr bool LEAN_TRACE = (NSP_ == 3) && (DIM_ == 3);
   static constexpr bool LEAN_ONE_HEX = LEAN_TRACE && !TWOT && TRANSPORT == TRANSPORT_ARGON_MINIMAL;
+  static constexpr bool STORED_GEOM = LEAN_ONE_HEX;
   static constexpr bool LAUNDER_FLUX = false;
   static constexpr int minw_grad(int dim, int p, int nc) {
     return (LEAN_TRACE && dim == 3 && !nc && p <= 3) ? TPSRHS_PLASMA_MINW_GRAD_LEAN : MINW_GRAD;
diff --git a/tps_amd/csrc/plasma_family.hpp b/tps_amd/csrc/plasma_family.hpp
--- a/tps_amd/csrc/plasma_family.hpp
+++ b/tps_amd/csrc/plasma_family.hpp
@@ -24,7 +24,10 @@
 #ifndef TPSRHS_PLASMA_HIGH_ORDERS
     case 1: op->launch = &launch_all<DIM, 1, PH>; break;
     case 2: op->launch = &launch_all<DIM, 2, PH>; break;
-    case 3: op->launch = &launch_all<DIM, 3, PH>; break;
+    case 3:
+      op->launch = &launch_all<DIM, 3, PH>;
+      if constexpr (GeomTab<Cfg<DIM, 3, 0>, PH>::ON) op->build_geom = &build_geometry<DIM, 3, PH>;
+      break;
 #else
     case 4: op->launch = &launch_all<DIM, 4, PH>; break;
     case 5: op->launch = &launch_all<DIM, 5, PH>; break;
@@ -74,6 +77,14 @@
 }
 #endif
 
+extern "C" void tpsrhs_family_layout(int *version, unsigned *op_bytes, unsigned *rk_bytes, unsigned *mesh_bytes) {
+  const LayoutStamp st = layout_stamp();
+  *version = st.version;
+  *op_bytes = st.op_bytes;
+  *rk_bytes = st.rk_bytes;
+  *mesh_bytes = st.mesh_bytes;
+}
+
 #define TPSRHS_PLASMA_FAMILY(name, DIM, NVEL, NSP, AMBI)                                                              \
   extern "C" int name(tpsrhs_operator *op, int two_temperature, int transport, char *err, int errlen) {               \
     auto say = [&](const char *what) {                                                                                \
diff --git a/tps_amd/csrc/tpsrhs.hip b/tps_amd/csrc/tpsrhs.hip
--- a/tps_amd/csrc/tpsrhs.hip
+++ b/tps_amd/csrc/tpsrhs.hip
@@ -52,6 +52,22 @@
       const std::string sym = "pick_" + unit;
       auto fn = reinterpret_cast<family_pick_fn>(dlsym(h, sym.c_str()));
       if (!fn) throw std::runtime_error(path + " does not export " + sym);
+      typedef void (*layout_fn)(int *, unsigned *, unsigned *, unsigned *);
+      auto lf = reinterpret_cast<layout_fn>(dlsym(h, "tpsrhs_family_layout"));
+      const LayoutStamp mine = layout_stamp();
+      LayoutStamp its = {0, 0, 0, 0};
+      if (lf) lf(&its.version, &its.op_bytes, &its.rk_bytes, &its.mesh_bytes);
+      if (!lf || its.version != mine.version || its.op_bytes != mine.op_bytes || its.rk_bytes != mine.rk_bytes ||
+          its.mesh_bytes != mine.mesh_bytes) {
+        dlclose(h);
+        throw Unsupported(path + " was built against another layout of the operator object (" +
+                          (lf ? "version " + std::to_string(its.version) + ", operator " + std::to_string(its.op_bytes) + " bytes, RkDev " +
+                                    std::to_string(its.rk_bytes) + ", MeshDev " + std::to_string(its.mesh_bytes)
+                              : std::string("no layout stamp")) +
+                          "; this library: version " + std::to_string(mine.version) + ", operator " + std::to_string(mine.op_bytes) +
+                          " bytes, RkDev " + std::to_string(mine.rk_bytes) + ", MeshDev " + std::to_string(mine.mesh_bytes) +
+                          "): rebuild the family and the core library from one source tree");
+      }
       loaded[unit] = fn;
       return fn;
     }
@@ -495,6 +511,7 @@
   }
 
   op->d_verts = dev_upload(tp.verts);
+  if (op->build_geom) op->build_geom(op);
   if (op->nc) op->d_minv = dev_upload(inverse_mass_matrices(tp.verts, op->dim, op->order, op->ne));
   {
     std::vector<int2> fi(tp.face_nbr.size());
@@ -1033,6 +1050,18 @@
   });
 }
 
+int64_t tpsrhs_geometry_table(tpsrhs_handle h, double *host_out, int64_t capacity, int *layout) {
+  if (!h || !h->d_geom) return 0;
+  const int64_t total = static_cast<int64_t>(h->ne) * h->geom_layout[0];
+  if (layout) std::memcpy(layout, h->geom_layout, sizeof h->geom_layout);
+  if (host_out && capacity >= total) {
+    if (hipSetDevice(h->device) != hipSuccess || hipStreamSynchronize(h->stream) != hipSuccess ||
+        hipMemcpy(host_out, h->d_geom, sizeof(double) * total, hipMemcpyDeviceToHost) != hipSuccess)
+      return -1;
+  }
+  return total;
+}
+
 int64_t tpsrhs_height(tpsrhs_handle h) { return h ? h->neq * h->ndofs : -1; }
 int64_t tpsrhs_num_dofs(tpsrhs_handle h) { return h ? h->ndofs : -1; }
 int tpsrhs_num_equation(tpsrhs_handle h) { return h ? h->neq : -1; }
diff --git a/tps_amd/rhs_operator.py b/tps_amd/rhs_operator.py
--- a/tps_amd/rhs_operator.py
+++ b/tps_amd/rhs_operator.py
@@ -94,6 +94,17 @@
             raise TpsRhsError(st, "tpsrhs_get_gradients")
         return out.view(self.dim, self.num_equation, self.NDofs)
 
+    def geometryTable(self):
+        layout = (C.c_int * 8)()
+        n = int(self._lib.tpsrhs_geometry_table(self._h, None, 0, layout))
+        if n <= 0:
+            return None, None
+        out = np.empty(n, dtype=np.float64)
+        got = int(self._lib.tpsrhs_geometry_table(self._h, out.ctypes.data_as(C.c_void_p), n, layout))
+        if got != n:
+            raise TpsRhsError(got, "tpsrhs_geometry_table")
+        return out.reshape(-1, layout[0]), list(layout)
+
     def getPlasmaConductivity(self, x: torch.Tensor) -> torch.Tensor:
         self._check(x)
         out = torch.empty(self.NDofs, dtype=torch.float64, device=self.device)
```

After: 12270. 0.965x the previous value.
